# nchopin/particles

Hardware: NVIDIA H100
Metric: particle-steps/sec (N x T), Bootstrap SV (higher is better)
Workload: dtype f64

## Files before the change

include/smcb.h:

```cpp
#ifndef SMCB_H
#define SMCB_H

#include <stdint.h>

#ifdef __cplusplus
extern "C" {
#endif

#define SMCB_OK 0
#define SMCB_EINVAL (-1)
#define SMCB_ECUDA (-2)
#define SMCB_ENOSYS (-3)

typedef struct smcb_ctx smcb_ctx;

const char *smcb_last_error(void);
int smcb_version(void);

int smcb_create(smcb_ctx **out, int device, uint64_t seed);
int smcb_destroy(smcb_ctx *ctx);
int smcb_set_stream(smcb_ctx *ctx, void *cuda_stream);
int smcb_seed(smcb_ctx *ctx, uint64_t seed);
int64_t smcb_launch_count(const smcb_ctx *ctx);


int smcb_normalise(smcb_ctx *ctx, double *lw, int64_t n, double *W_out, double *stats_out);
int smcb_weights_from_stats(smcb_ctx *ctx, const double *lw, int64_t n, const double *stats, double *W_out);

#define SMCB_LSE_SUM 0
#define SMCB_LSE_MEAN 1
#define SMCB_LSE_ESSL 2
int smcb_lse(smcb_ctx *ctx, int mode, const double *v, const double *W, int64_t n,
             double *out);

int smcb_exp_and_normalise(smcb_ctx *ctx, const double *lw, int64_t n, double *W_out);

int smcb_wmean_and_var(smcb_ctx *ctx, const double *W, const double *x, int64_t n, int d,
                       double *out);

#define SMCB_RS_MULTINOMIAL 0
#define SMCB_RS_STRATIFIED 1
#define SMCB_RS_SYSTEMATIC 2
#define SMCB_RS_RESIDUAL 3
#define SMCB_RS_SSP 4

int smcb_cumsum(smcb_ctx *ctx, const double *w, int64_t n, double *cdf_out);

int smcb_searchsorted(smcb_ctx *ctx, const double *cdf, int64_t n, const double *su,
                      int64_t m, int64_t *A_out);

int64_t smcb_resample_scratch_doubles(int64_t n, int64_t m);
int smcb_resample(smcb_ctx *ctx, int scheme, const double *W, int64_t n, int64_t m,
                  int64_t *A_out, const double *u_in, double *scratch);

int smcb_gather(smcb_ctx *ctx, const double *X, int64_t n, const int64_t *A, int64_t m,
                int d, double *Xp);
int smcb_gather_rows(smcb_ctx *ctx, const double *X, int64_t n, const int64_t *A, int64_t m,
                     int d, double *Xp);

int smcb_normal_rvs(smcb_ctx *ctx, const double *loc, double loc0, const double *scale,
                    double scale0, const double *z_in, double *out, int64_t n);
int smcb_normal_logpdf(smcb_ctx *ctx, const double *x, double x0, const double *loc,
                       double loc0, const double *scale, double scale0, double *out,
                       int64_t n);
int smcb_logpdf1(smcb_ctx *ctx, int kind, const double *x, double x0, double p0, double c0, const double *p1,
                 double p10, const double *p2, double p20, double *out, int64_t n);
int smcb_mvnormal_rvs(smcb_ctx *ctx, const double *loc, const double *loc0,
                      const double *scale, const double *scale0, const double *L, int d,
                      const double *z_in, double *out, int64_t n);
int smcb_mvnormal_logpdf(smcb_ctx *ctx, const double *x, const double *loc,
                         const double *loc0, const double *scale, const double *scale0,
                         const double *L, int d, double *out, int64_t n);
int smcb_standard_normal(smcb_ctx *ctx, double *out, int64_t n);
int smcb_uniform(smcb_ctx *ctx, double *out, int64_t n);

int smcb_logistic_target(smcb_ctx *ctx, const double *theta, int64_t n, int d, const double *data,
                         int64_t n_data, double prior_scale, double epn, double *lprior,
                         double *llik, double *lpost);
int smcb_rw_propose(smcb_ctx *ctx, const double *theta, int64_t n, int d, const double *L_dev,
                    const double *z_in, double *prop);
int smcb_mh_accept(smcb_ctx *ctx, int64_t n, int d, double *theta, double *lprior, double *llik,
                   double *lpost, const double *theta_p, const double *lprior_p, const double *llik_p,
                   const double *lpost_p, const double *u_in, double *mean_acc);

int smcb_logistic_wf_move(smcb_ctx *ctx, int64_t M, int d, int P, const double *theta0,
                          const double *lprior0, const double *llik0, const double *lpost0,
                          const double *data, int64_t n_data, double prior_scale, double epn,
                          const double *L_dev, const double *z_in, const double *u_in,
                          double *theta_out, double *lprior_out, double *llik_out, double *lpost_out,
                          double *pb_out);

int smcb_next_annealing_epn(smcb_ctx *ctx, const double *llik, int64_t n, double epn, double alpha, double *out_dev);
int smcb_rw_calibrate(smcb_ctx *ctx, const double *W, const double *theta, int64_t n, int d, double scale,
                      double *L_out);

int smcb_essl_grid(smcb_ctx *ctx, const double *llik, int64_t n, double lo, double hi, const double *max_dev,
                   double *out32_dev);
int smcb_wcov_sums(smcb_ctx *ctx, const double *W, const double *theta, int64_t n, int d, const double *mean_dev,
                   double *out_dev);
int smcb_chol_from_sums(smcb_ctx *ctx, const double *tri_dev, const double *sw_dev, int d, double scale, double *L_out);

int smcb_device_math(smcb_ctx *ctx, int fn, const double *x, double *out, int64_t n);

#define SMCB_FK_BOOTSTRAP 0
#define SMCB_FK_GUIDED 1
#define SMCB_FK_APF 2
#define SMCB_FK_AUXBOOT 3

#define SMCB_MODEL_STOCHVOL 0
#define SMCB_MODEL_LINGAUSS 1
#define SMCB_MODEL_GORDON 2
#define SMCB_MODEL_THETALOGISTIC 3
#define SMCB_MODEL_BEARINGS 4
#define SMCB_MODEL_MVLINGAUSS 5
#define SMCB_MODEL_DISCRETECOX 6
#define SMCB_MODEL_STOCHVOLLEV 7

#define SMCB_MAX_PARAMS 256
#define SMCB_SUMMARY_STRIDE 4

typedef struct smcb_filter smcb_filter;

typedef struct {
    int32_t model, fk, scheme, dim;
    int32_t dy, n_params;
    int32_t world, rank;
    int64_t n;
    int64_t n_global;
    int64_t index_offset;
    int64_t T;
    double essrmin;
    uint64_t seed;
    double params[SMCB_MAX_PARAMS];
    double *X[2];
    double *lw[2];
    int64_t *A;
    double *cdf;
    double *data;
    double *summaries;
    const double *z_in;
    const double *u_in;
    double *scratch;
    const double *step_consts;
    double *local_stats;
    const double *gathered;
    double *mail_local;
    double *mail_peer[8];
    int32_t rs_global, reserved0;
    double *moments;
    double *reserved1;
    const double *peer_X0[8];
    const double *peer_X1[8];
    const double *peer_cdf[8];
} smcb_filter_desc;

int smcb_filter_create(smcb_ctx *ctx, const smcb_filter_desc *desc, smcb_filter **out);
int smcb_filter_destroy(smcb_filter *f);
int smcb_filter_step(smcb_filter *f, int64_t nsteps);
int smcb_filter_step_local(smcb_filter *f);
int smcb_filter_step_finish(smcb_filter *f);
int smcb_p2p_alloc(smcb_ctx *ctx, int64_t bytes, void **dev_ptr, unsigned char *handle64);
int smcb_p2p_open(smcb_ctx *ctx, const unsigned char *handle64, void **dev_ptr);
int smcb_p2p_close(void *peer_ptr);
int smcb_p2p_free(void *dev_ptr);
int smcb_filter_step_timed(smcb_filter *f, int64_t nsteps, double *out8);
int smcb_filter_state(smcb_filter *f, double *out8);

#define SMCB_SMOOTH_ON2 0
#define SMCB_SMOOTH_MCMC 1
#define SMCB_SMOOTH_REJECT 2
#define SMCB_SMOOTH_GATHER 3

typedef struct {
    int32_t method, model, dim, n_params;
    int64_t T, N, M;
    int64_t nsteps;
    int64_t max_trials;
    double params[SMCB_MAX_PARAMS];
    const double *step_consts;
    const double *const *X;
    const double *const *lw;
    const int64_t *const *A;
    int64_t x_stride_n, x_stride_c;
    const double *log_bound;
    const double *cdf;
    int64_t cdf_ld;
    const int64_t *idx_T;
    const double *u;
    const int64_t *prop;
    const double *lu;
    const double *u_exact;
    int64_t *idx;
    double *paths;
    int64_t *counts;
} smcb_smooth_desc;

int smcb_backward_sample(smcb_ctx *ctx, const smcb_smooth_desc *desc);

#ifdef __cplusplus
}
#endif
#endif
```

particles_b200/_lib.py:

```python
import ctypes as C
import os

HERE = os.path.dirname(os.path.abspath(__file__))
SO_PATH = os.environ.get("SMCB_LIB") or os.path.join(HERE, "libsmcb.so")

SMCB_MAX_PARAMS = 256
SUMMARY_STRIDE = 4

RS_CODES = {"multinomial": 0, "stratified": 1, "systematic": 2, "residual": 3, "ssp": 4}
FUSED_SCHEMES = ("multinomial", "stratified", "systematic")
FK_BOOTSTRAP, FK_GUIDED, FK_APF, FK_AUXBOOT = 0, 1, 2, 3
MODEL_STOCHVOL, MODEL_LINGAUSS, MODEL_GORDON, MODEL_THETALOGISTIC = 0, 1, 2, 3
MODEL_BEARINGS, MODEL_MVLINGAUSS, MODEL_DISCRETECOX, MODEL_STOCHVOLLEV = 4, 5, 6, 7
LSE_SUM, LSE_MEAN, LSE_ESSL = 0, 1, 2

c_dp = C.c_void_p


class FilterDesc(C.Structure):
    _fields_ = [
        ("model", C.c_int32), ("fk", C.c_int32), ("scheme", C.c_int32), ("dim", C.c_int32),
        ("dy", C.c_int32), ("n_params", C.c_int32), ("world", C.c_int32), ("rank", C.c_int32),
        ("n", C.c_int64), ("n_global", C.c_int64), ("index_offset", C.c_int64), ("T", C.c_int64),
        ("essrmin", C.c_double), ("seed", C.c_uint64),
        ("params", C.c_double * SMCB_MAX_PARAMS),
        ("X", c_dp * 2), ("lw", c_dp * 2), ("A", c_dp), ("cdf", c_dp), ("data", c_dp),
        ("summaries", c_dp), ("z_in", c_dp), ("u_in", c_dp), ("scratch", c_dp),
        ("step_consts", c_dp), ("local_stats", c_dp), ("gathered", c_dp),
        ("mail_local", c_dp), ("mail_peer", c_dp * 8),
        ("rs_global", C.c_int32), ("reserved0", C.c_int32), ("moments", c_dp), ("reserved1", c_dp),
        ("peer_X0", c_dp * 8), ("peer_X1", c_dp * 8), ("peer_cdf", c_dp * 8),
    ]


SMOOTH_ON2, SMOOTH_MCMC, SMOOTH_REJECT, SMOOTH_GATHER = 0, 1, 2, 3


class SmoothDesc(C.Structure):
    _fields_ = [
        ("method", C.c_int32), ("model", C.c_int32), ("dim", C.c_int32), ("n_params", C.c_int32),
        ("T", C.c_int64), ("N", C.c_int64), ("M", C.c_int64), ("nsteps", C.c_int64), ("max_trials", C.c_int64),
        ("params", C.c_double * SMCB_MAX_PARAMS), ("step_consts", c_dp),
        ("X", c_dp), ("lw", c_dp), ("A", c_dp), ("x_stride_n", C.c_int64), ("x_stride_c", C.c_int64),
        ("log_bound", c_dp), ("cdf", c_dp), ("cdf_ld", C.c_int64), ("idx_T", c_dp),
        ("u", c_dp), ("prop", c_dp), ("lu", c_dp), ("u_exact", c_dp),
        ("idx", c_dp), ("paths", c_dp), ("counts", c_dp),
    ]


PROTOTYPES = {
    "smcb_last_error": (C.c_char_p, []),
    "smcb_version": (C.c_int, []),
    "smcb_create": (C.c_int, [C.POINTER(C.c_void_p), C.c_int, C.c_uint64]),
    "smcb_destroy": (C.c_int, [C.c_void_p]),
    "smcb_set_stream": (C.c_int, [C.c_void_p, C.c_void_p]),
    "smcb_seed": (C.c_int, [C.c_void_p, C.c_uint64]),
    "smcb_launch_count": (C.c_int64, [C.c_void_p]),
    "smcb_normalise": (C.c_int, [C.c_void_p, c_dp, C.c_int64, c_dp, c_dp]),
    "smcb_weights_from_stats": (C.c_int, [C.c_void_p, c_dp, C.c_int64, c_dp, c_dp]),
    "smcb_lse": (C.c_int, [C.c_void_p, C.c_int, c_dp, c_dp, C.c_int64, c_dp]),
    "smcb_exp_and_normalise": (C.c_int, [C.c_void_p, c_dp, C.c_int64, c_dp]),
    "smcb_wmean_and_var": (C.c_int, [C.c_void_p, c_dp, c_dp, C.c_int64, C.c_int, c_dp]),
    "smcb_cumsum": (C.c_int, [C.c_void_p, c_dp, C.c_int64, c_dp]),
    "smcb_searchsorted": (C.c_int, [C.c_void_p, c_dp, C.c_int64, c_dp, C.c_int64, c_dp]),
    "smcb_resample_scratch_doubles": (C.c_int64, [C.c_int64, C.c_int64]),
    "smcb_resample": (C.c_int, [C.c_void_p, C.c_int, c_dp, C.c_int64, C.c_int64, c_dp, c_dp, c_dp]),
    "smcb_gather": (C.c_int, [C.c_void_p, c_dp, C.c_int64, c_dp, C.c_int64, C.c_int, c_dp]),
    "smcb_gather_rows": (C.c_int, [C.c_void_p, c_dp, C.c_int64, c_dp, C.c_int64, C.c_int, c_dp]),
    "smcb_normal_rvs": (C.c_int, [C.c_void_p, c_dp, C.c_double, c_dp, C.c_double, c_dp, c_dp, C.c_int64]),
    "smcb_normal_logpdf": (C.c_int, [C.c_void_p, c_dp, C.c_double, c_dp, C.c_double, c_dp, C.c_double,
                                     c_dp, C.c_int64]),
    "smcb_logpdf1": (C.c_int, [C.c_void_p, C.c_int, c_dp, C.c_double, C.c_double, C.c_double, c_dp, C.c_double, c_dp,
                               C.c_double, c_dp, C.c_int64]),
    "smcb_mvnormal_rvs": (C.c_int, [C.c_void_p, c_dp, c_dp, c_dp, c_dp, c_dp, C.c_int, c_dp, c_dp, C.c_int64]),
    "smcb_mvnormal_logpdf": (C.c_int, [C.c_void_p, c_dp, c_dp, c_dp, c_dp, c_dp, c_dp, C.c_int, c_dp,
                                       C.c_int64]),
    "smcb_standard_normal": (C.c_int, [C.c_void_p, c_dp, C.c_int64]),
    "smcb_uniform": (C.c_int, [C.c_void_p, c_dp, C.c_int64]),
    "smcb_logistic_target": (C.c_int, [C.c_void_p, c_dp, C.c_int64, C.c_int, c_dp, C.c_int64, C.c_double,
                                       C.c_double, c_dp, c_dp, c_dp]),
    "smcb_logistic_wf_move": (C.c_int, [C.c_void_p, C.c_int64, C.c_int, C.c_int, c_dp, c_dp, c_dp, c_dp, c_dp,
                                        C.c_int64, C.c_double, C.c_double, c_dp, c_dp, c_dp, c_dp, c_dp, c_dp,
                                        c_dp, c_dp]),
    "smcb_rw_propose": (C.c_int, [C.c_void_p, c_dp, C.c_int64, C.c_int, c_dp, c_dp, c_dp]),
    "smcb_mh_accept": (C.c_int, [C.c_void_p, C.c_int64, C.c_int, c_dp, c_dp, c_dp, c_dp, c_dp, c_dp, c_dp, c_dp,
                                 c_dp, c_dp]),
    "smcb_next_annealing_epn": (C.c_int, [C.c_void_p, c_dp, C.c_int64, C.c_double, C.c_double, c_dp]),
    "smcb_rw_calibrate": (C.c_int, [C.c_void_p, c_dp, c_dp, C.c_int64, C.c_int, C.c_double, c_dp]),
    "smcb_essl_grid": (C.c_int, [C.c_void_p, c_dp, C.c_int64, C.c_double, C.c_double, c_dp, c_dp]),
    "smcb_wcov_sums": (C.c_int, [C.c_void_p, c_dp, c_dp, C.c_int64, C.c_int, c_dp, c_dp]),
    "smcb_chol_from_sums": (C.c_int, [C.c_void_p, c_dp, c_dp, C.c_int, C.c_double, c_dp]),
    "smcb_device_math": (C.c_int, [C.c_void_p, C.c_int, c_dp, c_dp, C.c_int64]),
    "smcb_filter_create": (C.c_int, [C.c_void_p, C.POINTER(FilterDesc), C.POINTER(C.c_void_p)]),
    "smcb_filter_destroy": (C.c_int, [C.c_void_p]),
    "smcb_filter_step": (C.c_int, [C.c_void_p, C.c_int64]),
    "smcb_filter_step_local": (C.c_int, [C.c_void_p]),
    "smcb_filter_step_finish": (C.c_int, [C.c_void_p]),
    "smcb_p2p_alloc": (C.c_int, [C.c_void_p, C.c_int64, C.POINTER(C.c_void_p), C.c_char_p]),
    "smcb_p2p_open": (C.c_int, [C.c_void_p, C.c_char_p, C.POINTER(C.c_void_p)]),
    "smcb_p2p_close": (C.c_int, [C.c_void_p]),
    "smcb_p2p_free": (C.c_int, [C.c_void_p]),
    "smcb_filter_step_timed": (C.c_int, [C.c_void_p, C.c_int64, C.POINTER(C.c_double)]),
    "smcb_filter_state": (C.c_int, [C.c_void_p, C.POINTER(C.c_double)]),
    "smcb_backward_sample": (C.c_int, [C.c_void_p, C.POINTER(SmoothDesc)]),
}

_lib = None


class SmcbError(RuntimeError):
    pass


def load():
    global _lib
    if _lib is None:
        if not os.path.exists(SO_PATH):
            raise SmcbError(
                f"{SO_PATH} is missing: build it with `python -m particles_b200.build` "
                "(there is no CPU fallback for this path)")
        lib = C.CDLL(SO_PATH)
        for name, (res, args) in PROTOTYPES.items():
            fn = getattr(lib, name)
            fn.restype, fn.argtypes = res, args
        _lib = lib
    return _lib


def check(rc):
    if rc == 0:
        return
    msg = load().smcb_last_error().decode()
    if rc == -1:
        raise ValueError(msg)
    if rc == -3:
        raise NotImplementedError(msg)
    raise SmcbError(msg)
```

particles_b200/core.py:

```python
import ctypes as C
import time

import numpy as np
import torch

from . import _lib
from . import collectors
from . import resampling as rs
from .device import as_device, context, empty, ptr, require_cuda, tensor_from_ptr


class FeynmanKac:

    def __init__(self, T):
        self.T = T

    def _error_msg(self, meth):
        return f"method/property {meth} missing in class {self.__class__.__name__}"

    def M0(self, N):
        raise NotImplementedError(self._error_msg("M0"))

    def M(self, t, xp):
        raise NotImplementedError(self._error_msg("M"))

    def logG(self, t, xp, x):
        raise NotImplementedError(self._error_msg("logG"))

    @property
    def isAPF(self):
        return "logeta" in dir(self)

    def done(self, smc):
        return smc.t >= self.T

    def time_to_resample(self, smc):
        return smc.aux.ESS < smc.N * smc.ESSrmin

    def default_moments(self, W, X):
        return rs.wmean_and_var(W, X)

    def summary_format(self, smc):
        return "t=%i: resample:%s, ESS (end of iter)=%.2f" % (smc.t, smc.rs_flag, smc.wgts.ESS)


def _is_apf(fk):
    return fk.isAPF if hasattr(fk, "isAPF") else ("logeta" in dir(fk))


class _FusedEngine:

    def __init__(self, spec, N, scheme, ESSrmin, seed, noise=None, n_global=None, index_offset=0,
                 world=1, rank=0, group=None, p2p=False, global_rs=False, moments=False):
        self.world, self.rank, self.group = int(world), int(rank), group
        self.p2p = bool(p2p) and self.world > 1
        self.global_rs = bool(global_rs) and self.world > 1
        if self.global_rs and not self.p2p:
            raise ValueError("global resampling over shards needs the peer-memory exchange (exchange='p2p')")
        self._pool = None
        self.ctx = context()
        self.lib = self.ctx.lib
        self.N, self.T = int(N), int(spec["data"].shape[0])
        n, T = self.N, self.T
        self.dim, self.dy = int(spec.get("dim", 1)), int(spec.get("dy", 1))
        dev = self.ctx.device
        f64 = dict(dtype=torch.float64, device=dev)
        xshape = (n,) if self.dim == 1 else (self.dim, n)
        if self.p2p:
            self._pool = _p2p_pool(self.ctx, self.world, self.rank, group)
        if self.global_rs:
            arena = self._pool.arena((2 * self.dim + 1) * n * 8)
            nd = self.dim * n
            self.X = [tensor_from_ptr(arena, xshape, owner=self._pool), tensor_from_ptr(arena + nd * 8, xshape, owner=self._pool)]
            self.cdf = tensor_from_ptr(arena + 2 * nd * 8, (n,), owner=self._pool)
        else:
            self.X = [torch.empty(xshape, **f64), torch.empty(xshape, **f64)]
            self.cdf = torch.empty(n, **f64)
        self.lw = [torch.empty(n, **f64), torch.empty(n, **f64)]
        self.A = torch.empty(n, dtype=torch.int64, device=dev)
        self.summ = torch.zeros((T, _lib.SUMMARY_STRIDE), **f64)
        self.mom = torch.zeros((T, 8), **f64) if moments else None
        self.data_host = torch.from_numpy(spec["data"].reshape(-1)).pin_memory()
        self.data = self.data_host.to(dev, non_blocking=True)
        self.sc = None
        if spec.get("step_consts") is not None:
            self.sc = as_device(spec["step_consts"])
        self.scratch = torch.empty(n + 2, **f64) if scheme == "multinomial" else None
        self.z_in = self.u_in = None
        if noise is not None:
            z, u = noise
            self.z_in = None if z is None else as_device(z)
            self.u_in = None if u is None else as_device(u)
        d = _lib.FilterDesc()
        d.model, d.fk, d.scheme, d.dim = spec["model"], spec["fk"], _lib.RS_CODES[scheme], self.dim
        d.dy, d.n_params = self.dy, len(spec["params"])
        d.n, d.n_global = n, int(n_global or n)
        d.index_offset, d.T = int(index_offset), T
        d.essrmin, d.seed = float(ESSrmin), int(seed) & (2 ** 64 - 1)
        for i, v in enumerate(spec["params"]):
            d.params[i] = float(v)
        d.X[0], d.X[1] = self.X[0].data_ptr(), self.X[1].data_ptr()
        d.lw[0], d.lw[1] = self.lw[0].data_ptr(), self.lw[1].data_ptr()
        d.A, d.cdf = self.A.data_ptr(), self.cdf.data_ptr()
        d.data, d.summaries = self.data.data_ptr(), self.summ.data_ptr()
        d.z_in = self.z_in.data_ptr() if self.z_in is not None else None
        d.u_in = self.u_in.data_ptr() if self.u_in is not None else None
        d.scratch = self.scratch.data_ptr() if self.scratch is not None else None
        d.step_consts = self.sc.data_ptr() if self.sc is not None else None
        d.moments = self.mom.data_ptr() if self.mom is not None else None
        d.world, d.rank = self.world, self.rank
        if self.world > 1:
            self.local_stats = torch.zeros(16, **f64)
            self.gathered = torch.zeros(16 * self.world, **f64)
            d.local_stats, d.gathered = self.local_stats.data_ptr(), self.gathered.data_ptr()
            if self.p2p:
                mail = self._pool.mailbox()
                d.mail_local = mail[self.rank]
                for r in range(self.world):
                    d.mail_peer[r] = mail[r]
            if self.global_rs:
                nd = self.dim * n * 8
                d.rs_global = 1
                for r in range(self.world):
                    base = self._pool.arena_of(r)
                    d.peer_X0[r], d.peer_X1[r], d.peer_cdf[r] = base, base + nd, base + 2 * nd
        self.desc = d
        h = C.c_void_p()
        _lib.check(self.lib.smcb_filter_create(self.ctx.handle, C.byref(d), C.byref(h)))
        self.handle = h

    def step(self, nsteps=1):
        self.ctx.bind_stream()
        if self.world == 1 or self.p2p:
            _lib.check(self.lib.smcb_filter_step(self.handle, int(nsteps)))
            return
        import torch.distributed as dist
        for _ in range(int(nsteps)):
            _lib.check(self.lib.smcb_filter_step_local(self.handle))
            dist.all_gather_into_tensor(self.gathered, self.local_stats, group=self.group)
            _lib.check(self.lib.smcb_filter_step_finish(self.handle))

    def step_timed(self, nsteps):
        self.ctx.bind_stream()
        out = (C.c_double * 8)()
        _lib.check(self.lib.smcb_filter_step_timed(self.handle, int(nsteps), out))
        ms = dict(zip(("init", "step_rs", "tail", "step"), out[0:4]))
        cnt = dict(zip(("init", "step_rs", "tail", "step"), (int(v) for v in out[4:8])))
        return ms, cnt

    def state(self):
        out = (C.c_double * 8)()
        _lib.check(self.lib.smcb_filter_state(self.handle, out))
        return list(out)

    def close(self):
        if getattr(self, "handle", None):
            self.lib.smcb_filter_destroy(self.handle)
            self.handle = None

    def __del__(self):
        try:
            self.close()
        except Exception:
            pass


class _P2PPool:

    def __init__(self, ctx, world, rank, group):
        self.ctx, self.lib, self.world, self.rank, self.group = ctx, ctx.lib, world, rank, group
        self._mail = None
        self._arena = None
        self._arena_bytes = 0
        self._gen = 0

    def _exchange(self, nbytes):
        import torch.distributed as dist
        ptr_ = C.c_void_p()
        hbuf = C.create_string_buffer(64)
        _lib.check(self.lib.smcb_p2p_alloc(self.ctx.handle, int(nbytes), C.byref(ptr_), hbuf))
        mine = torch.frombuffer(bytearray(hbuf.raw), dtype=torch.uint8).to(self.ctx.device)
        allh = torch.empty(64 * self.world, dtype=torch.uint8, device=self.ctx.device)
        dist.all_gather_into_tensor(allh, mine, group=self.group)
        allh = allh.cpu().numpy().tobytes()
        out = []
        for r in range(self.world):
            if r == self.rank:
                out.append(ptr_.value)
                continue
            pp = C.c_void_p()
            _lib.check(self.lib.smcb_p2p_open(self.ctx.handle, allh[64 * r:64 * (r + 1)], C.byref(pp)))
            out.append(pp.value)
        return out

    def mailbox(self):
        nslab, slab = 4, 2 * self.world * 32 * 8
        if self._mail is None:
            self._mail = self._exchange(nslab * slab)
        g = self._gen
        self._gen += 1
        tensor_from_ptr(self._mail[self.rank] + ((g + 2) % nslab) * slab, (slab // 8,), owner=self).zero_()
        return [p + (g % nslab) * slab for p in self._mail]

    def arena(self, nbytes):
        if self._arena is None or nbytes > self._arena_bytes:
            self._arena = self._exchange(nbytes)
            self._arena_bytes = nbytes
        return self._arena[self.rank]

    def arena_of(self, r):
        return self._arena[r]


_pools = {}


def _p2p_pool(ctx, world, rank, group):
    key = (ctx.device.index, id(group) if group is not None else None, world, rank)
    if key not in _pools:
        _pools[key] = _P2PPool(ctx, world, rank, group)
    return _pools[key]


class SMC:

    def __init__(self, fk=None, N=100, qmc=False, resampling="systematic", ESSrmin=0.5,
                 store_history=False, verbose=False, collect=None, seed=None, fused=None,
                 noise=None):
        require_cuda()
        _lib.load()
        if qmc:
            raise NotImplementedError("SQMC (qmc=True) is outside the accelerated path")
        if resampling not in rs.rs_funcs:
            raise ValueError(f"{resampling} is not a valid resampling scheme")
        self.fk, self.N, self.qmc = fk, N, qmc
        self.resampling, self.ESSrmin, self.verbose = resampling, ESSrmin, verbose
        self.t = 0
        self._done = 0
        self.cpu_time = None
        self.summaries = None if collect == "off" else collectors.Summaries(collect)
        self._seed = np.random.randint(0, 2 ** 31 - 1) if seed is None else int(seed)
        self._engine = None
        self._dev_moments = False
        self._noise = noise
        spec = None
        if fused is not False:
            from .state_space_models import fused_spec
            spec = fused_spec(fk)
            if spec is not None and resampling not in _lib.FUSED_SCHEMES:
                spec = None
            if spec is None and fused is True:
                raise NotImplementedError("this Feynman-Kac model has no fused kernel")
        if spec is not None:
            self._dev_moments = self.summaries is not None and self.summaries.device_moments(fk)
            self._engine = _FusedEngine(spec, N, resampling, ESSrmin, self._seed, noise,
                                        moments=self._dev_moments)
            self._row_cache = {}
        else:
            context().seed(self._seed)
            self._p = {"rs_flag": False, "logLt": 0.0, "wgts": rs.Weights(), "aux": None,
                       "X": None, "Xp": None, "A": None}
        from . import smoothing
        self.hist = smoothing.generate_hist_obj(store_history, self)

    @property
    def fused(self):
        return self._engine is not None

    def _row(self, t):
        if t not in self._row_cache:
            self._row_cache = {t: self._engine.summ[t].cpu().numpy()}
        return self._row_cache[t]

    def _cur(self):
        return (self._done - 1) & 1

    @property
    def X(self):
        if not self.fused:
            return self._p["X"]
        if self._done == 0:
            return None
        x = self._engine.X[self._cur()]
        return x if x.ndim == 1 else x.t()

    @X.setter
    def X(self, v):
        self._p["X"] = v

    @property
    def rs_flag(self):
        if not self.fused:
            return self._p["rs_flag"]
        return False if self._done == 0 else bool(self._row(self._done - 1)[2])

    @property
    def logLt(self):
        if not self.fused:
            return self._p["logLt"]
        return 0.0 if self._done == 0 else float(self._row(self._done - 1)[1])

    @property
    def log_mean_w(self):
        if not self.fused:
            return self._p["log_mean_w"]
        return float(self._row(self._done - 1)[3])

    @property
    def loglt(self):
        if not self.fused:
            return self._p["loglt"]
        t = self._done - 1
        if t == 0 or self.rs_flag:
            return self.log_mean_w
        return self.log_mean_w - float(self._engine.summ[t - 1, 3].item())

    @property
    def A(self):
        if not self.fused:
            return self._p["A"]
        if self._done <= 1:
            return None
        if self.rs_flag:
            return self._engine.A
        return torch.arange(self.N, device=self._engine.A.device)

    @property
    def Xp(self):
        if not self.fused:
            return self._p["Xp"]
        if self._done <= 1:
            return None
        prev = self._engine.X[self._cur() ^ 1]
        if not self.rs_flag:
            return prev if prev.ndim == 1 else prev.t()
        out = torch.empty_like(prev)
        ctx = self._engine.ctx
        _lib.check(ctx.lib.smcb_gather(ctx.handle, ptr(prev), self.N, ptr(self._engine.A), self.N,
                                       self._engine.dim, ptr(out)))
        return out if out.ndim == 1 else out.t()

    @property
    def wgts(self):
        if not self.fused:
            return self._p["wgts"]
        if self._done == 0:
            return rs.Weights()
        st = self._engine.state()
        stats = torch.tensor([st[6], st[5], st[4], st[7]], dtype=torch.float64,
                             device=self._engine.lw[0].device)
        return rs.Weights._from_device_stats(self._engine.lw[self._cur()], stats)

    @property
    def aux(self):
        if not self.fused:
            return self._p["aux"]
        return self.wgts

    @property
    def W(self):
        return self.wgts.W

    def __str__(self):
        return self.fk.summary_format(self)

    def reset_weights(self):
        p = self._p
        if _is_apf(self.fk):
            lw = rs.log_mean_exp(self.logetat, W=p["wgts"].W) - self._gather(self.logetat, p["A"])
            p["wgts"] = rs.Weights(lw=lw)
        else:
            p["wgts"] = rs.Weights()

    def setup_auxiliary_weights(self):
        p = self._p
        if _is_apf(self.fk):
            self.logetat = as_device(self.fk.logeta(self.t - 1, p["X"]))
            p["aux"] = p["wgts"].add(self.logetat)
        else:
            p["aux"] = p["wgts"]

    def _gather(self, X, A):
        if not isinstance(X, (torch.Tensor, np.ndarray)):
            return X[A]
        ctx = context()
        X = as_device(X)
        d = 1 if X.ndim == 1 else X.shape[1]
        out = torch.empty((A.shape[0],) + tuple(X.shape[1:]), dtype=X.dtype, device=X.device)
        _lib.check(ctx.lib.smcb_gather_rows(ctx.handle, ptr(X), X.shape[0], ptr(A), A.shape[0], d,
                                            ptr(out)))
        return out

    def generate_particles(self):
        self._p["X"] = self.fk.M0(self.N)

    def reweight_particles(self):
        p = self._p
        p["wgts"] = p["wgts"].add(self.fk.logG(self.t, p["Xp"], p["X"]))

    def resample_move(self):
        p = self._p
        p["rs_flag"] = bool(self.fk.time_to_resample(self))
        if p["rs_flag"]:
            p["A"] = rs.resampling(self.resampling, p["aux"].W, M=self.N)
            p["Xp"] = self._gather(p["X"], p["A"])
            self.reset_weights()
        else:
            p["A"] = torch.arange(self.N, device="cuda")
            p["Xp"] = p["X"]
        p["X"] = self.fk.M(self.t, p["Xp"])

    def compute_summaries(self):
        p = self._p
        if self.t > 0:
            prec = p["log_mean_w"]
        p["log_mean_w"] = p["wgts"].log_mean
        if self.t == 0 or p["rs_flag"]:
            p["loglt"] = p["log_mean_w"]
        else:
            p["loglt"] = p["log_mean_w"] - prec
        p["logLt"] += p["loglt"]
        if self.verbose:
            print(self)
        if self.hist:
            self.hist.save(self)
        if self.summaries:
            self.summaries.collect(self)

    def __next__(self):
        if self.fk.done(self):
            raise StopIteration
        if self.fused:
            self._engine.step(1)
            self._done += 1
            if self.verbose:
                print(self)
            if self.hist:
                self.hist.save(self)
            if self.summaries:
                self.summaries.collect(self)
            self.t += 1
            return
        if self.t == 0:
            self.generate_particles()
        else:
            self.setup_auxiliary_weights()
            self.resample_move()
        self.reweight_particles()
        self.compute_summaries()
        self.t += 1
        self._done = self.t

    def next(self):
        return self.__next__()

    def __iter__(self):
        return self

    def run(self):
        t0 = time.perf_counter()
        if self.fused and not self.verbose and not self.hist \
                and (self.summaries is None or self.summaries.only_defaults or self._dev_moments) \
                and getattr(getattr(type(self.fk), "done", None), "__qualname__", "") == "FeynmanKac.done":
            T = self._engine.T
            first = self.t
            if first < T:
                self._engine.step(T - first)
                self.t = self._done = T
            table = self._engine.summ.cpu().numpy()
            self._row_cache = {T - 1: table[T - 1]}
            if self.summaries is not None:
                self.summaries._extend_defaults([float(v) for v in table[first:T, 0]],
                                                [float(v) for v in table[first:T, 1]],
                                                [bool(v) for v in table[first:T, 2]])
                if self._dev_moments:
                    self.summaries._extend_moments(self._engine.mom.cpu().numpy()[first:T], self._engine.dim)
        else:
            for _ in self:
                pass
            if self.fused:
                torch.cuda.synchronize()
        self.cpu_time = time.perf_counter() - t0
```

particles_b200/csrc/smcb_filter.cu:

```cuda
#include <stdlib.h>

#include "smcb_step.cuh"

int smcb_bind_nd(smcb_filter *f);
int smcb_bind_1d_more(smcb_filter *f);

static int smcb_bind_1d(smcb_filter *f) {
    const smcb_filter_desc *d = &f->desc;
    switch (d->model) {
        case SMCB_MODEL_STOCHVOL: return bind_fk<StochVolM>(f);
        case SMCB_MODEL_LINGAUSS: return bind_fk<LinGaussM>(f);
        case SMCB_MODEL_GORDON:
        case SMCB_MODEL_THETALOGISTIC:
        case SMCB_MODEL_DISCRETECOX:
        case SMCB_MODEL_STOCHVOLLEV: return smcb_bind_1d_more(f);
        default:
            set_error("fused filter: model id %d is not available in the fused 1-D family", d->model);
            return SMCB_ENOSYS;
    }
}

static int filter_setup(smcb_filter *f, smcb_ctx *c, const smcb_filter_desc *d);

extern "C" int smcb_filter_create(smcb_ctx *c, const smcb_filter_desc *d, smcb_filter **out) {
    SMCB_REQUIRE(c && d && out, "smcb_filter_create: NULL argument");
    SMCB_REQUIRE(d->n >= 1 && d->T >= 1, "smcb_filter_create: need n >= 1 and T >= 1");
    SMCB_REQUIRE(d->X[0] && d->X[1] && d->lw[0] && d->lw[1] && d->A && d->cdf && d->data && d->summaries,
                 "smcb_filter_create: NULL device buffer");
    SMCB_REQUIRE((d->index_offset & 1) == 0, "smcb_filter_create: index_offset must be even");
    SMCB_REQUIRE(d->dim >= 1 && d->dim <= 4, "smcb_filter_create: fused kernels exist for state dimension 1..4 (dim=%d)", d->dim);
    SMCB_REQUIRE(d->dy >= 1 && d->dy <= kMaxDy, "smcb_filter_create: observation dimension must be 1..%d", kMaxDy);
    SMCB_REQUIRE(d->essrmin >= 0.0 && d->essrmin <= 1.0, "smcb_filter_create: ESSrmin must be in [0, 1]");
    smcb_filter *f = new (std::nothrow) smcb_filter();
    SMCB_REQUIRE(f != nullptr, "smcb_filter_create: out of host memory");
    f->ctx = c;
    f->desc = *d;
    f->t_host = 0;
    f->timed = false;
    f->mem = nullptr;
    const int rc = filter_setup(f, c, d);
    if (rc) {
        if (f->mem) cudaFree(f->mem);
        delete f;
        return rc;
    }
    *out = f;
    return SMCB_OK;
}

static bool env_flag(const char *name, bool dflt) {
    const char *v = getenv(name);
    if (!v || !*v) return dflt;
    return v[0] != '0';
}

static int filter_setup(smcb_filter *f, smcb_ctx *c, const smcb_filter_desc *d) {
    int rc = (d->dim == 1) ? smcb_bind_1d(f) : smcb_bind_nd(f);
    if (rc) return rc;

    const int64_t n = d->n;
    constexpr size_t kHdr = 512;
    static_assert(2 * sizeof(StepState) <= 384, "StepState outgrew its header slot");
    const size_t part = (size_t)2 * kMaxStepGrid * kPartStride * sizeof(double);
    const size_t agg = (size_t)(kMaxStepGrid + 8) * sizeof(double);
    SMCB_CUDA(cudaMalloc(&f->mem, kHdr + part + agg));
    SMCB_CUDA(cudaMemsetAsync(f->mem, 0, kHdr + part + agg, c->stream));
    FilterArgs &a = f->args;
    memset(&a, 0, sizeof(a));
    a.st = reinterpret_cast<StepState *>(f->mem);
    a.bar = reinterpret_cast<unsigned long long *>(f->mem + 384);
    a.sync_timeout = reinterpret_cast<int *>(f->mem + 392);
    a.partials = reinterpret_cast<double *>(f->mem + kHdr);
    a.blk_agg = reinterpret_cast<double *>(f->mem + kHdr + part);
    a.math_tab = c->math_tab;
    a.X[0] = d->X[0]; a.X[1] = d->X[1]; a.lw[0] = d->lw[0]; a.lw[1] = d->lw[1];
    a.A = reinterpret_cast<long long *>(d->A);
    a.cdf = d->cdf;
    a.su = (d->scheme == SMCB_RS_MULTINOMIAL) ? d->scratch : nullptr;
    SMCB_REQUIRE(d->scheme != SMCB_RS_MULTINOMIAL || d->scratch != nullptr,
                 "smcb_filter_create: multinomial needs desc.scratch of n + 2 doubles");
    a.data = d->data;
    a.sc = d->step_consts;
    a.summaries = d->summaries;
    a.moments = d->moments;
    a.z_in = d->z_in; a.u_in = d->u_in;
    a.dy = d->dy;
    a.n = n; a.n_global = d->n_global > 0 ? d->n_global : n;
    a.index_offset = d->index_offset; a.T = d->T;
    a.essrmin = d->essrmin;
    a.key = key_of(d->seed);
    {
        int dev = 0, sms = kSMs;
        SMCB_CUDA(cudaGetDevice(&dev));
        SMCB_CUDA(cudaDeviceGetAttribute(&sms, cudaDevAttrMultiProcessorCount, dev));
        const int64_t npairs = (n + 1) / 2;
        int64_t g = sms < kMaxStepGrid ? sms : kMaxStepGrid;
        const int64_t gmax = (npairs + f->block_size - 1) / f->block_size;
        if (g > gmax) g = gmax;
        if (g < 1) g = 1;
        int64_t chunk = (npairs + g - 1) / g;
        g = (npairs + chunk - 1) / chunk;
        a.chunk = chunk;
        f->grid_move = (int)g;
        a.grid = f->grid_move;
        const bool apf = d->fk == SMCB_FK_APF || d->fk == SMCB_FK_AUXBOOT;
        const bool mom = d->moments != nullptr;
        a.slab_lane = (!apf && !mom) ? 1 : 0;
        a.slab_stride = a.slab_lane ? 96 : 4 + (apf ? 4 : 0) + (mom ? 2 * d->dim : 0);
        const int64_t cap = f->slab_doubles / a.slab_stride;
        const int64_t n_iter = (chunk + f->pairs_per_iteration - 1) / f->pairs_per_iteration;
        int64_t slab_it = 2, n_small = 0;
        for (;; slab_it++) {
            const int64_t ns = (cap * slab_it - n_iter) / (slab_it - 1) - 1;
            const int64_t want = n_iter < 32 ? n_iter : 32;
            if (ns >= want) { n_small = ns < 0 ? 0 : (ns > n_iter / 8 ? n_iter / 8 : ns); break; }
        }
        if (n_small > n_iter) n_small = n_iter;
        a.slab_it = (int)slab_it;
        a.slab_small = (int)n_small;
    }
    a.world = d->world > 1 ? d->world : 1;
    a.rank = d->world > 1 ? d->rank : 0;
    a.local_stats = d->local_stats;
    a.gathered = d->gathered;
    a.mail_local = (a.world > 1) ? d->mail_local : nullptr;
    for (int r = 0; r < 8; r++) a.mail_peer[r] = (a.world > 1 && r < a.world) ? d->mail_peer[r] : nullptr;
    SMCB_REQUIRE(a.world == 1 || (a.rank >= 0 && a.rank < a.world), "smcb_filter_create: bad rank");
    SMCB_REQUIRE(a.world == 1 || a.mail_local || (d->local_stats && d->gathered),
                 "smcb_filter_create: world > 1 needs either a peer mailbox or local_stats / gathered");
    SMCB_REQUIRE(a.world <= 8, "smcb_filter_create: at most 8 ranks");
    if (a.mail_local) {
        for (int r = 0; r < a.world; r++)
            SMCB_REQUIRE(a.mail_peer[r] != nullptr, "smcb_filter_create: mail_peer[%d] is NULL", r);
    }
    a.rs_global = (a.world > 1 && d->rs_global) ? 1 : 0;
    if (a.rs_global) {
        SMCB_REQUIRE(a.mail_local != nullptr, "smcb_filter_create: global resampling needs the peer mailbox");
        SMCB_REQUIRE((n & 1) == 0, "smcb_filter_create: global resampling needs an even shard size");
        if (d->scheme != SMCB_RS_SYSTEMATIC && d->scheme != SMCB_RS_STRATIFIED) {
            set_error("fused filter: global resampling over shards supports systematic and stratified");
            return SMCB_ENOSYS;
        }
        for (int r = 0; r < a.world; r++) {
            SMCB_REQUIRE(d->peer_X0[r] && d->peer_X1[r] && d->peer_cdf[r],
                         "smcb_filter_create: peer_X0 / peer_X1 / peer_cdf[%d] is NULL", r);
            a.pX[r][0] = d->peer_X0[r]; a.pX[r][1] = d->peer_X1[r]; a.pcdf[r] = d->peer_cdf[r];
        }
    }
    f->pdl = env_flag("SMCB_PDL", true);
    f->coop = env_flag("SMCB_COOP", false);
    return SMCB_OK;
}

extern "C" int smcb_filter_destroy(smcb_filter *f) {
    if (!f) return SMCB_OK;
    cudaStreamSynchronize(f->ctx->stream);
    cudaFree(f->mem);
    delete f;
    return SMCB_OK;
}

static int launch_one(smcb_filter *f) {
    if (f->t_host >= f->desc.T) {
        set_error("smcb_filter_step: all %lld steps already done (StopIteration)", (long long)f->desc.T);
        return SMCB_EINVAL;
    }
    int rc = (f->t_host == 0) ? f->launch_init(f) : f->launch_step(f);
    if (rc && f->t_host > 0 && (f->pdl || f->coop)) {
        cudaGetLastError();
        f->pdl = false; f->coop = false;
        rc = f->launch_step(f);
    }
    if (rc) return rc;
    f->t_host++;
    return SMCB_OK;
}

extern "C" int smcb_filter_step_local(smcb_filter *f) {
    SMCB_REQUIRE(f != nullptr && f->args.world > 1 && f->args.mail_local == nullptr,
                 "smcb_filter_step_local: not a sharded filter with the host-driven exchange");
    int rc = launch_one(f);
    if (rc) return rc;
    return f->launch_publish(f);
}

extern "C" int smcb_filter_step_finish(smcb_filter *f) {
    SMCB_REQUIRE(f != nullptr && f->args.world > 1, "smcb_filter_step_finish: not a sharded filter");
    return f->launch_tail(f);
}

extern "C" int smcb_filter_step(smcb_filter *f, int64_t nsteps) {
    SMCB_REQUIRE(f != nullptr, "smcb_filter_step: NULL filter");
    SMCB_REQUIRE(f->args.world == 1 || f->args.mail_local != nullptr,
                 "smcb_filter_step: sharded filters without a peer mailbox use step_local / step_finish");
    if (nsteps <= 0) return SMCB_OK;
    for (int64_t i = 0; i < nsteps; i++) {
        int rc = launch_one(f);
        if (rc) return rc;
    }
    return f->launch_tail(f);
}

extern "C" int smcb_filter_step_timed(smcb_filter *f, int64_t nsteps, double *out8) {
    SMCB_REQUIRE(f && out8, "smcb_filter_step_timed: NULL argument");
    SMCB_REQUIRE(nsteps >= 1 && nsteps <= 100000, "smcb_filter_step_timed: nsteps out of range");
    SMCB_REQUIRE(f->t_host + nsteps <= f->desc.T, "smcb_filter_step_timed: past the last step");
    SMCB_REQUIRE(f->args.world == 1, "smcb_filter_step_timed: single-device filters only");
    cudaStream_t s = f->ctx->stream;
    const size_t nev = (size_t)(nsteps + 1) * 2;
    cudaEvent_t *ev = new (std::nothrow) cudaEvent_t[nev];
    double *rows = new (std::nothrow) double[(size_t)nsteps * SMCB_SUMMARY_STRIDE];
    size_t made = 0;
    int rc = SMCB_OK;
    const int64_t t_first = f->t_host;
    auto fail = [&](cudaError_t e, const char *what) {
        set_error("smcb_filter_step_timed: %s -> %s", what, cudaGetErrorString(e));
        rc = SMCB_ECUDA;
    };
    if (!ev || !rows) { set_error("smcb_filter_step_timed: out of host memory"); rc = SMCB_EINVAL; }
    for (; rc == SMCB_OK && made < nev; made++) {
        cudaError_t e = cudaEventCreate(&ev[made]);
        if (e != cudaSuccess) { fail(e, "cudaEventCreate"); break; }
    }
    f->timed = true;
    for (int64_t i = 0; rc == SMCB_OK && i <= nsteps; i++) {
        cudaEventRecord(ev[2 * i], s);
        rc = (i < nsteps) ? launch_one(f) : f->launch_tail(f);
        cudaEventRecord(ev[2 * i + 1], s);
    }
    f->timed = false;
    if (rc == SMCB_OK) {
        cudaError_t e = cudaStreamSynchronize(s);
        if (e != cudaSuccess) fail(e, "cudaStreamSynchronize");
    }
    if (rc == SMCB_OK) {
        cudaError_t e = cudaMemcpy(rows, f->args.summaries + (size_t)t_first * SMCB_SUMMARY_STRIDE,
                                   sizeof(double) * nsteps * SMCB_SUMMARY_STRIDE, cudaMemcpyDeviceToHost);
        if (e != cudaSuccess) fail(e, "cudaMemcpy(summaries)");
    }
    if (rc == SMCB_OK) {
        for (int j = 0; j < 8; j++) out8[j] = 0.0;
        for (int64_t i = 0; i <= nsteps; i++) {
            float ms = 0.f;
            cudaEventElapsedTime(&ms, ev[2 * i], ev[2 * i + 1]);
            int kind = 2;
            if (i < nsteps) {
                const int64_t t = t_first + i;
                kind = (t == 0) ? 0 : (rows[(size_t)i * SMCB_SUMMARY_STRIDE + 2] != 0.0 ? 1 : 3);
            }
            out8[kind] += ms;
            out8[4 + kind] += 1.0;
        }
    }
    for (size_t i = 0; i < made; i++) cudaEventDestroy(ev[i]);
    delete[] ev;
    delete[] rows;
    return rc;
}

extern "C" int smcb_filter_state(smcb_filter *f, double *out8) {
    SMCB_REQUIRE(f && out8, "smcb_filter_state: NULL argument");
    SMCB_REQUIRE(f->t_host >= 1, "smcb_filter_state: no step has run yet");
    struct { StepState st[2]; char pad[384 - 2 * sizeof(StepState)]; unsigned long long bar; int timeout; int pad2; } h;
    static_assert(sizeof(h) == 400, "header snapshot layout");
    SMCB_CUDA(cudaMemcpyAsync(&h, f->mem, sizeof(h), cudaMemcpyDeviceToHost, f->ctx->stream));
    SMCB_CUDA(cudaStreamSynchronize(f->ctx->stream));
    const StepState &s = h.st[(f->t_host - 1) & 1];
    out8[0] = (double)(s.t + 1); out8[1] = (double)((f->t_host - 1) & 1); out8[2] = (double)s.rs; out8[3] = s.logLt;
    out8[4] = s.ess; out8[5] = s.log_mean_w; out8[6] = s.wm; out8[7] = s.ws;
    if (h.timeout) {
        set_error(h.timeout == 2 ? "fused filter: the grid barrier of a resampling step timed out (the step kernel was "
                                   "not co-resident: another kernel occupies the device)"
                                 : "sharded filter: a wait on a peer GPU's flag timed out (a rank died or fell out of step)");
        return SMCB_ECUDA;
    }
    if (s.t != f->t_host - 1) {
        set_error("smcb_filter_state: the last step is not finalised (internal error: t=%lld, expected %lld)",
                  (long long)s.t, (long long)(f->t_host - 1));
        return SMCB_ECUDA;
    }
    return SMCB_OK;
}

extern "C" int smcb_p2p_alloc(smcb_ctx *c, int64_t bytes, void **dev_ptr, unsigned char *handle64) {
    SMCB_REQUIRE(c && dev_ptr && handle64 && bytes > 0, "smcb_p2p_alloc: bad argument");
    static_assert(sizeof(cudaIpcMemHandle_t) == 64, "IPC handle size");
    void *p = nullptr;
    SMCB_CUDA(cudaMalloc(&p, (size_t)bytes));
    SMCB_CUDA(cudaMemset(p, 0, (size_t)bytes));
    cudaIpcMemHandle_t h;
    SMCB_CUDA(cudaIpcGetMemHandle(&h, p));
    memcpy(handle64, &h, 64);
    *dev_ptr = p;
    return SMCB_OK;
}

extern "C" int smcb_p2p_open(smcb_ctx *c, const unsigned char *handle64, void **dev_ptr) {
    SMCB_REQUIRE(c && dev_ptr && handle64, "smcb_p2p_open: bad argument");
    cudaIpcMemHandle_t h;
    memcpy(&h, handle64, 64);
    SMCB_CUDA(cudaIpcOpenMemHandle(dev_ptr, h, cudaIpcMemLazyEnablePeerAccess));
    return SMCB_OK;
}

extern "C" int smcb_p2p_close(void *peer_ptr) {
    if (peer_ptr) SMCB_CUDA(cudaIpcCloseMemHandle(peer_ptr));
    return SMCB_OK;
}

extern "C" int smcb_p2p_free(void *dev_ptr) {
    if (dev_ptr) SMCB_CUDA(cudaFree(dev_ptr));
    return SMCB_OK;
}
```

particles_b200/csrc/smcb_step.cuh:

```cuda
#pragma once
#include <string.h>

#include <new>

#include "smcb_common.cuh"
#include "smcb_math.cuh"
#include "smcb_models.cuh"
#include "smcb_scan.cuh"
#include "smcb_search.cuh"

using namespace smcb;

namespace smcb {

constexpr int kPartStride = 16;
constexpr int kMailStride = 32;
constexpr int kMailEpoch = 16;
constexpr int kMailScan = 17;
constexpr int kMaxStepGrid = 256;
constexpr int kMaxD = 4;
constexpr int kTailBlock = 256;
#ifndef SMCB_SPECULATE
#define SMCB_SPECULATE 1
#endif
template <class M> struct StepCfg {
    static constexpr int BS = 512;
    static constexpr int kU = (M::D == 1) ? 2 : 1;
    static constexpr int kStage = 8 * BS;
    static constexpr int kSlabRecords = 128;
    static constexpr int kSlabDoubles = kSlabRecords * 96;
    static constexpr size_t dyn_smem = kMathTabBytes + (size_t)(2 * kStage > kSlabDoubles ? 2 * kStage : kSlabDoubles) * sizeof(double);
};
constexpr int kScanGroupWarps = 2;
constexpr int kMovePairs = 2;

struct StepState {
    double logLt, log_mean_w, ess;
    double wm, ws, wq;
    long long t;
    long long nrs;
    int rs;
    int rs_next;
    int pad[2];
};

struct FilterArgs {
    double *X[2];
    double *lw[2];
    long long *A;
    double *cdf;
    double *su;
    const double *data;
    const double *sc;
    double *summaries;
    double *moments;
    const double *z_in, *u_in;
    StepState *st;
    int *sync_timeout;
    double *partials;
    unsigned long long *bar;
    double *blk_agg;
    const double *math_tab;
    int slab_it;
    int slab_small;
    int slab_lane;
    int slab_stride;
    int64_t n, n_global, index_offset, T;
    int dy;
    int world, rank;
    int grid;
    int64_t chunk;
    double essrmin;
    Philox key;
    double *local_stats;
    const double *gathered;
    double *mail_local;
    double *mail_peer[8];
    int rs_global;
    const double *pX[8][2];
    const double *pcdf[8];
};

__device__ __forceinline__ void wait_epoch(const volatile double *flag, double epoch, int *timeout) {
    const long long t0 = clock64();
    if (*reinterpret_cast<volatile int *>(timeout)) return;
    while (*flag < epoch) {
        if (clock64() - t0 > 8000000000ll) { *timeout = 1; break; }
    }
    __threadfence_system();
}

__device__ __forceinline__ StepK step_consts(const FilterArgs &a, long long t) {
    StepK k;
    k.t = t;
#pragma unroll
    for (int i = 0; i < kMaxDy; i++) {
        k.yv[i] = (i < a.dy && t >= 0) ? a.data[t * a.dy + i] : 0.0;
        k.yn[i] = (i < a.dy && t + 1 < a.T) ? a.data[(t + 1) * a.dy + i] : 0.0;
    }
    k.y = k.yv[0];
    k.y_next = k.yn[0];
    k.sc0 = (a.sc && t >= 0) ? a.sc[t] : 0.0;
    return k;
}

__device__ __forceinline__ double fix_nan(double v) { return v != v ? -CUDART_INF : v; }

__device__ __forceinline__ void weights_scalars(const Lse3 &a, double n, double &log_mean, double &ess) {
    if (a.m == -CUDART_INF || a.m == CUDART_INF || a.m != a.m) {
        log_mean = CUDART_NAN;
        ess = CUDART_NAN;
        return;
    }
    log_mean = a.m + log(a.s / n);
    ess = (a.s * a.s) / a.q;
}

__device__ __forceinline__ double shift_factor(double m, double M) {
    return (m == -CUDART_INF) ? 0.0 : fexp_neg(m - M);
}

__device__ __forceinline__ double nanmax(double a, double b) { return (b > a || b != b) ? b : a; }

template <int NV, int BS, bool MAX>
__device__ __forceinline__ void block_reduce_all(double (&v)[NV], double *smem) {
    constexpr int NWARP = BS / 32;
    static_assert(NWARP <= 32, "one lane per warp in the second level");
    const int lane = threadIdx.x & 31, warp = threadIdx.x >> 5;
#pragma unroll
    for (int j = 0; j < NV; j++) {
#pragma unroll
        for (int mask = 16; mask > 0; mask >>= 1) {
            const double o = __shfl_xor_sync(0xffffffffu, v[j], mask);
            v[j] = MAX ? nanmax(v[j], o) : v[j] + o;
        }
    }
    if (lane == 0) {
#pragma unroll
        for (int j = 0; j < NV; j++) smem[warp * NV + j] = v[j];
    }
    __syncthreads();
    if (warp == 0) {
#pragma unroll
        for (int j = 0; j < NV; j++) {
            double x = (lane < NWARP) ? smem[lane * NV + j] : (MAX ? -CUDART_INF : 0.0);
#pragma unroll
            for (int mask = 16; mask > 0; mask >>= 1) {
                const double o = __shfl_xor_sync(0xffffffffu, x, mask);
                x = MAX ? nanmax(x, o) : x + o;
            }
            if (lane == 0) smem[NWARP * NV + j] = x;
        }
    }
    __syncthreads();
#pragma unroll
    for (int j = 0; j < NV; j++) v[j] = smem[NWARP * NV + j];
    __syncthreads();
}
template <int NV, int BS>
__device__ __forceinline__ void block_max_all(double (&v)[NV], double *smem) { block_reduce_all<NV, BS, true>(v, smem); }
template <int NV, int BS>
__device__ __forceinline__ void block_sum_all(double (&v)[NV], double *smem) { block_reduce_all<NV, BS, false>(v, smem); }

template <int D>
struct Acc {
    Lse3 w;
    double sx[D], sxx[D];
};

template <int D>
__device__ __forceinline__ void acc_init(Acc<D> &a) {
    a.w = lse3_empty();
#pragma unroll
    for (int c = 0; c < D; c++) { a.sx[c] = 0.0; a.sxx[c] = 0.0; }
}

template <int NV, int D, bool FINITE, bool MOM>
__device__ __forceinline__ void acc_add_batch_t(Acc<D> &a, const double (&v)[NV], const double (&x)[NV][D]) {
    double mb = v[0];
#pragma unroll
    for (int j = 1; j < NV; j++) mb = FINITE ? (v[j] > mb ? v[j] : mb) : fmax(mb, v[j]);
    if (mb > a.w.m) {
        const double r = texp_neg(a.w.m - mb);
        a.w.s *= r;
        a.w.q *= r * r;
        if (MOM) {
#pragma unroll
            for (int c = 0; c < D; c++) { a.sx[c] *= r; a.sxx[c] *= r; }
        }
        a.w.m = mb;
    }
    if (!FINITE && a.w.m == -CUDART_INF) return;
#pragma unroll
    for (int j = 0; j < NV; j++) {
        const double e = FINITE ? texp_sat(v[j] - a.w.m) : texp_neg(v[j] - a.w.m);
        a.w.s += e;
        a.w.q = fma(e, e, a.w.q);
        if (MOM && (FINITE || v[j] != -CUDART_INF)) {
#pragma unroll
            for (int c = 0; c < D; c++) {
                const double ex = e * x[j][c];
                a.sx[c] += ex;
                a.sxx[c] = fma(ex, x[j][c], a.sxx[c]);
            }
        }
    }
}
template <int NV, int D, bool FINITE = false>
__device__ __forceinline__ void acc_add_batch(Acc<D> &a, const double (&v)[NV], const double (&x)[NV][D], bool mom) {
    if (mom) acc_add_batch_t<NV, D, FINITE, true>(a, v, x);
    else acc_add_batch_t<NV, D, FINITE, false>(a, v, x);
}

struct StepSmem {
    double red[32 * 16];
    int next;
    double ringP[32];
    int ringF[32];
    double gwarp[16][8];
    double gpref[16][2];
    int gqn[16];
    long long gq[16][8][3];
    int *timeout_ptr;
    double peer[8][kMailStride];
    double goff[9], gpi[8];
    double pref[2];
    double carry[20];
};

__device__ __forceinline__ double shift_factor_t(double m, double M) {
    return (m == -CUDART_INF) ? 0.0 : texp_neg(m - M);
}

__device__ __forceinline__ double warp_max_nan(double v) {
#pragma unroll
    for (int mask = 16; mask > 0; mask >>= 1) {
        const double o = __shfl_xor_sync(0xffffffffu, v, mask);
        v = (o > v || o != o) ? o : v;
    }
    return v;
}
__device__ __forceinline__ double warp_sum(double v) {
#pragma unroll
    for (int mask = 16; mask > 0; mask >>= 1) v += __shfl_xor_sync(0xffffffffu, v, mask);
    return v;
}

template <int D, bool APF>
__device__ __forceinline__ void warp_reduce_to_slab(const Acc<D> &sa, const Lse3 &sx, bool mom, double *rec, int lane) {
    const double M = warp_max_nan(sa.w.m);
    const double e = shift_factor_t(sa.w.m, M);
    const double s = warp_sum(sa.w.s * e), q = warp_sum(sa.w.q * (e * e));
    if (lane == 0) { rec[0] = M; rec[1] = s; rec[2] = q; }
    int off = 4;
    if (APF) {
        const double Ma = warp_max_nan(sx.m);
        const double ea = shift_factor_t(sx.m, Ma);
        const double as_ = warp_sum(sx.s * ea), aq = warp_sum(sx.q * (ea * ea));
        if (lane == 0) { rec[4] = Ma; rec[5] = as_; rec[6] = aq; }
        off = 8;
    }
    if (mom) {
#pragma unroll
        for (int c = 0; c < D; c++) {
            const double a1 = warp_sum(sa.sx[c] * e), a2 = warp_sum(sa.sxx[c] * e);
            if (lane == 0) { rec[off + c] = a1; rec[off + D + c] = a2; }
        }
    }
}

template <int D, bool APF, int BS>
__device__ __forceinline__ void write_partial(const FilterArgs &a, long long t, const Acc<D> &acc, const Lse3 &aux,
                                              bool mom, StepSmem &sh, const double *s_slab = nullptr, int n_slab = 0) {
    const bool lane_rec = a.slab_lane != 0;
    const int n_rec = lane_rec ? n_slab * 32 : n_slab;
    auto rec_ptr = [&](int r) {
        return lane_rec ? s_slab + (size_t)(r >> 5) * a.slab_stride + (r & 31) : s_slab + (size_t)r * a.slab_stride;
    };
    const int rs_ = lane_rec ? 32 : 1;
    if (n_slab > 0) __syncthreads();
    double mx[2] = {acc.w.m, APF ? aux.m : -CUDART_INF};
    for (int r = threadIdx.x; r < n_rec; r += BS) {
        const double *rec = rec_ptr(r);
        mx[0] = nanmax(mx[0], rec[0]);
        if (APF && !lane_rec) mx[1] = nanmax(mx[1], rec[4]);
    }
    block_max_all<2, BS>(mx, sh.red);
    const double ew = shift_factor_t(acc.w.m, mx[0]);
    const double ea = APF ? shift_factor_t(aux.m, mx[1]) : 0.0;
    double v[4 + 2 * D];
    v[0] = acc.w.s * ew;
    v[1] = acc.w.q * (ew * ew);
    v[2] = APF ? aux.s * ea : 0.0;
    v[3] = APF ? aux.q * (ea * ea) : 0.0;
#pragma unroll
    for (int c = 0; c < D; c++) {
        v[4 + c] = mom ? acc.sx[c] * ew : 0.0;
        v[4 + D + c] = mom ? acc.sxx[c] * ew : 0.0;
    }
    for (int r = threadIdx.x; r < n_rec; r += BS) {
        const double *rec = rec_ptr(r);
        const double e = shift_factor_t(rec[0], mx[0]);
        v[0] += rec[rs_] * e;
        v[1] += rec[2 * rs_] * (e * e);
        if (!lane_rec) {
            if (APF) {
                const double e2 = shift_factor_t(rec[4], mx[1]);
                v[2] += rec[5] * e2;
                v[3] += rec[6] * (e2 * e2);
            }
            if (mom) {
                const int off = APF ? 8 : 4;
#pragma unroll
                for (int c = 0; c < D; c++) { v[4 + c] += rec[off + c] * e; v[4 + D + c] += rec[off + D + c] * e; }
            }
        }
    }
    if (mom) block_sum_all<4 + 2 * D, BS>(v, sh.red);
    else {
        double w4[4] = {v[0], v[1], v[2], v[3]};
        block_sum_all<4, BS>(w4, sh.red);
        v[0] = w4[0]; v[1] = w4[1]; v[2] = w4[2]; v[3] = w4[3];
    }
    if (threadIdx.x == 0) {
        double *p = a.partials + ((size_t)(t & 1) * kMaxStepGrid + blockIdx.x) * kPartStride;
        p[0] = mx[0]; p[1] = v[0]; p[2] = v[1]; p[3] = 0.0;
        p[4] = APF ? mx[1] : mx[0]; p[5] = APF ? v[2] : v[0]; p[6] = APF ? v[3] : v[1]; p[7] = 0.0;
#pragma unroll
        for (int c = 0; c < kMaxD; c++) {
            p[8 + c] = (c < D) ? v[4 + (c < D ? c : 0)] : 0.0;
            p[12 + c] = (c < D) ? v[4 + D + (c < D ? c : 0)] : 0.0;
        }
    }
}

__device__ __forceinline__ void merge16(double (&a)[16], const double *b) {
#pragma unroll
    for (int k = 0; k < 2; k++) {
        const double am = a[4 * k], bm = b[4 * k];
        const double M = (bm > am || bm != bm) ? bm : am;
        const double ea = shift_factor(am, M), eb = shift_factor(bm, M);
        a[4 * k] = M;
        a[4 * k + 1] = a[4 * k + 1] * ea + b[4 * k + 1] * eb;
        a[4 * k + 2] = a[4 * k + 2] * (ea * ea) + b[4 * k + 2] * (eb * eb);
        if (k == 0) {
#pragma unroll
            for (int c = 8; c < 16; c++) a[c] = a[c] * ea + b[c] * eb;
        }
    }
}

template <bool APF>
__device__ __forceinline__ void shard_totals(const FilterArgs &a, long long s, bool mom, StepSmem &sh, double (&loc)[16]) {
    const int G = a.grid, tid = threadIdx.x;
    if (tid < 32) {
        const double *base = a.partials + (size_t)(s & 1) * kMaxStepGrid * kPartStride;
        constexpr int kR = kMaxStepGrid / 32;
        double pm[kR], ps[kR], pq[kR], xm[kR], xs[kR], xq[kR];
        double mw = -CUDART_INF, ma = -CUDART_INF;
#pragma unroll
        for (int i = 0; i < kR; i++) {
            const int r = tid + 32 * i;
            pm[i] = -CUDART_INF; ps[i] = 0.0; pq[i] = 0.0; xm[i] = -CUDART_INF; xs[i] = 0.0; xq[i] = 0.0;
            if (r < G) {
                const double *row = base + (size_t)r * kPartStride;
                const double2 r0 = __ldcg(reinterpret_cast<const double2 *>(row));
                pm[i] = r0.x; ps[i] = r0.y; pq[i] = __ldcg(row + 2);
                if (APF) {
                    const double2 r1 = __ldcg(reinterpret_cast<const double2 *>(row + 4));
                    xm[i] = r1.x; xs[i] = r1.y; xq[i] = __ldcg(row + 6);
                }
            }
            mw = nanmax(mw, pm[i]);
            if (APF) ma = nanmax(ma, xm[i]);
        }
        mw = warp_max_nan(mw);
        if (APF) ma = warp_max_nan(ma);
        double v[12];
#pragma unroll
        for (int j2 = 0; j2 < 12; j2++) v[j2] = 0.0;
#pragma unroll
        for (int i = 0; i < kR; i++) {
            const int r = tid + 32 * i;
            const double ew = shift_factor(pm[i], mw);
            v[0] += ps[i] * ew;
            v[1] += pq[i] * (ew * ew);
            if (APF) {
                const double ea = shift_factor(xm[i], ma);
                v[2] += xs[i] * ea;
                v[3] += xq[i] * (ea * ea);
            }
            if (mom && r < G) {
                const double *row = base + (size_t)r * kPartStride + 8;
#pragma unroll
                for (int c = 0; c < 8; c++) v[4 + c] += __ldcg(row + c) * ew;
            }
        }
#pragma unroll
        for (int j2 = 0; j2 < 12; j2++)
            if (j2 < 4 || mom) v[j2] = warp_sum(v[j2]);
        if (tid == 0) {
            double *o = sh.peer[0];
            o[0] = mw; o[1] = v[0]; o[2] = v[1]; o[3] = 0.0;
            o[4] = APF ? ma : mw; o[5] = APF ? v[2] : v[0]; o[6] = APF ? v[3] : v[1]; o[7] = 0.0;
#pragma unroll
            for (int c = 0; c < 8; c++) o[8 + c] = v[4 + c];
        }
    }
    __syncthreads();
#pragma unroll
    for (int j2 = 0; j2 < 16; j2++) loc[j2] = sh.peer[0][j2];
    __syncthreads();
}

template <int BS>
__device__ __forceinline__ void cta_prefix(double v, StepSmem &sh, double &p_b, double &p_next) {
    const int tid = threadIdx.x, lane = tid & 31, warp = tid >> 5;
    const double iw = warp_scan_monotone(v, lane);
    if (lane == 31) sh.red[warp] = iw;
    __syncthreads();
    double woff = 0.0;
    for (int w_ = 0; w_ < BS / 32; w_++)
        if (w_ < warp) woff = woff + sh.red[w_];
    const double incl = woff + iw;
    if (tid == 0 && blockIdx.x == 0) sh.pref[0] = 0.0;
    if (tid + 1 == (int)blockIdx.x) sh.pref[0] = incl;
    if (tid == (int)blockIdx.x) sh.pref[1] = incl;
    __syncthreads();
    p_b = sh.pref[0];
    p_next = fmax(sh.pref[1], p_b);
    __syncthreads();
}

struct StepDecision {
    int rs;
    long long nrs_prev;
    double reset_c;
    double xm, xs;
    double p_b, p_next;
};

struct PrologueCarry {
    bool mom;
};

template <bool APF>
__device__ __forceinline__ bool prologue_begin(const FilterArgs &a, long long t, StepSmem &sh, bool writer,
                                               PrologueCarry &pc) {
    const long long s = t - 1;
    const int tid = threadIdx.x;
    pc.mom = writer && a.moments != nullptr;
    StepState prev;
    prev.logLt = 0.0; prev.log_mean_w = 0.0; prev.nrs = 0; prev.rs_next = 0;
    if (s >= 1) {
        const StepState *pp = a.st + ((s - 1) & 1);
        prev.logLt = __ldcg(&pp->logLt); prev.log_mean_w = __ldcg(&pp->log_mean_w);
        prev.nrs = __ldcg(&pp->nrs); prev.rs_next = __ldcg(&pp->rs_next);
    }
    double loc[16];
    shard_totals<APF>(a, s, pc.mom, sh, loc);
    if (tid == 0) {
#pragma unroll
        for (int i = 0; i < 16; i++) sh.carry[i] = loc[i];
        sh.carry[16] = prev.logLt; sh.carry[17] = prev.log_mean_w;
        sh.carry[18] = __longlong_as_double(prev.nrs); sh.carry[19] = __longlong_as_double((long long)prev.rs_next);
    }
    if (a.world > 1 && a.mail_local != nullptr) {
        if (writer && tid < a.world) {
            double *slot = a.mail_peer[tid] + ((size_t)(s & 1) * a.world + a.rank) * kMailStride;
#pragma unroll
            for (int i = 0; i < 16; i++) slot[i] = loc[i];
            __threadfence_system();
            *reinterpret_cast<volatile double *>(slot + kMailEpoch) = (double)(s + 1);
        }
    }
    const Lse3 xl{loc[4], loc[5], loc[6]};
    double lm_l, ess_l;
    weights_scalars(xl, (double)a.n, lm_l, ess_l);
    return (s + 1 < a.T) && (ess_l < (double)a.n * a.essrmin);
}

template <bool APF, int BS>
__device__ __forceinline__ StepDecision prologue_end(const FilterArgs &a, long long t, StepSmem &sh, bool writer,
                                                     bool need_prefix, const PrologueCarry &pc) {
    const long long s = t - 1;
    const int tid = threadIdx.x;
    __syncthreads();
    StepState prev;
    double loc[16];
#pragma unroll
    for (int i = 0; i < 16; i++) loc[i] = sh.carry[i];
    prev.logLt = sh.carry[16]; prev.log_mean_w = sh.carry[17];
    prev.nrs = __double_as_longlong(sh.carry[18]); prev.rs_next = (int)__double_as_longlong(sh.carry[19]);
    double glob[16];
#pragma unroll
    for (int j = 0; j < 16; j++) glob[j] = loc[j];
    if (a.world > 1) {
        if (a.mail_local != nullptr) {
            const double *box = a.mail_local + (size_t)(s & 1) * a.world * kMailStride;
            if (tid < a.world) {
                wait_epoch(box + (size_t)tid * kMailStride + kMailEpoch, (double)(s + 1), a.sync_timeout);
                for (int i = 0; i < 16; i++)
                    sh.peer[tid][i] = *reinterpret_cast<const volatile double *>(box + (size_t)tid * kMailStride + i);
            }
        } else if (tid < a.world) {
            for (int i = 0; i < 16; i++) sh.peer[tid][i] = __ldcg(a.gathered + (size_t)tid * 16 + i);
        }
        __syncthreads();
#pragma unroll
        for (int j = 0; j < 16; j++) glob[j] = sh.peer[0][j];
        for (int r = 1; r < a.world; r++) merge16(glob, sh.peer[r]);
        if (a.rs_global && tid == 0) {
            double run = 0.0;
            for (int r = 0; r < a.world; r++) {
                const double pm_ = sh.peer[r][4], ps_ = sh.peer[r][5];
                const double pi = (pm_ == -CUDART_INF) ? 0.0 : ps_ * fexp_neg(pm_ - glob[4]) / glob[5];
                sh.goff[r] = run;
                sh.gpi[r] = pi;
                run = run + pi;
            }
            sh.goff[a.world] = run;
        }
        __syncthreads();
    }
    const Lse3 w{glob[0], glob[1], glob[2]}, x{glob[4], glob[5], glob[6]};
    const Lse3 xl{loc[4], loc[5], loc[6]};
    const double N = (double)a.n_global;
    double log_mean, ess, lm_aux, ess_aux;
    weights_scalars(w, N, log_mean, ess);
    if (APF) weights_scalars(x, N, lm_aux, ess_aux);
    else { lm_aux = log_mean; ess_aux = ess; }
    const int rs_s = prev.rs_next;
    const bool fresh = (s == 0) || (rs_s != 0);
    const double loglt = fresh ? log_mean : (log_mean - prev.log_mean_w);
    const double logLt = prev.logLt + loglt;
    StepDecision d;
    d.rs = (s + 1 < a.T) && (ess_aux < N * a.essrmin);
    d.nrs_prev = prev.nrs + (rs_s ? 1 : 0);
    double rc = 0.0;
    if (a.rs_global) rc = APF ? (log(x.s) + x.m) - (log(w.s) + w.m) : 0.0;
    else if (APF || a.world > 1) rc = (log(xl.s) + xl.m) - (log(w.s) + w.m) + log((double)a.world);
    d.reset_c = rc;
    d.xm = xl.m; d.xs = xl.s;
    d.p_b = 0.0; d.p_next = 0.0;
    if (writer && tid == 0) {
        double *row = a.summaries + (size_t)s * SMCB_SUMMARY_STRIDE;
        row[0] = ess; row[1] = logLt; row[2] = (double)rs_s; row[3] = log_mean;
        StepState *o = a.st + (s & 1);
        o->logLt = logLt; o->log_mean_w = log_mean; o->ess = ess;
        o->wm = w.m; o->ws = w.s; o->wq = w.q;
        o->t = s; o->nrs = d.nrs_prev; o->rs = rs_s; o->rs_next = d.rs;
        if (a.moments != nullptr) {
            double *mrow = a.moments + (size_t)s * 2 * kMaxD;
#pragma unroll
            for (int c = 0; c < kMaxD; c++) {
                const double mean = glob[8 + c] / w.s;
                mrow[c] = mean;
                mrow[kMaxD + c] = glob[12 + c] / w.s - mean * mean;
            }
        }
    }
    if (d.rs && need_prefix) {
        double v = 0.0;
        if (tid < a.grid) {
            const double *row = a.partials + ((size_t)(s & 1) * kMaxStepGrid + tid) * kPartStride + (APF ? 4 : 0);
            v = __ldcg(row + 1) * shift_factor(__ldcg(row), d.xm) / d.xs;
        }
        cta_prefix<BS>(v, sh, d.p_b, d.p_next);
    }
    return d;
}

template <bool APF, int BS>
__device__ __forceinline__ StepDecision step_prologue(const FilterArgs &a, long long t, StepSmem &sh, bool writer,
                                                      bool need_prefix) {
    PrologueCarry pc;
    prologue_begin<APF>(a, t, sh, writer, pc);
    return prologue_end<APF, BS>(a, t, sh, writer, need_prefix, pc);
}

__device__ __forceinline__ void grid_barrier(const FilterArgs &a, unsigned long long target) {
    __syncthreads();
    if (threadIdx.x == 0) {
        __threadfence();
        atomicAdd(a.bar, 1ull);
        const long long t0 = clock64();
        while (*reinterpret_cast<volatile unsigned long long *>(a.bar) < target) {
            if (clock64() - t0 > 8000000000ll) { *a.sync_timeout = 2; break; }
        }
        __threadfence();
        asm volatile("fence.proxy.async;" ::: "memory");
    }
    __syncthreads();
}

__device__ __forceinline__ void cta_range(const FilterArgs &a, int64_t &pstart, int64_t &pend) {
    const int64_t npairs = (a.n + 1) >> 1;
    pstart = (int64_t)blockIdx.x * a.chunk;
    pend = pstart + a.chunk < npairs ? pstart + a.chunk : npairs;
    if (pstart > npairs) pstart = npairs;
}

template <class M, int FK>
__global__ void __launch_bounds__(StepCfg<M>::BS, 1) k_init(M model, FilterArgs a) {
    constexpr bool APF = FkTraits<FK>::apf;
    constexpr int D = M::D, NZ = M::NZ, BS = StepCfg<M>::BS;
    __shared__ StepSmem sh;
    __shared__ __align__(8) uint64_t s_tabbar;
    if (threadIdx.x == 0) mtab_issue(a.math_tab, &s_tabbar);
    __syncthreads();
    mbar_wait(&s_tabbar, 0);
    const StepK k = step_consts(a, 0);
    double *Xo = a.X[0], *lwo = a.lw[0];
    Acc<D> acc;
    acc_init(acc);
    Lse3 aux = lse3_empty();
    const bool mom = a.moments != nullptr;
    const int64_t n = a.n;
    const bool has_next = APF && a.T > 1;
    const bool vec_x = (D == 1) || ((n & 1) == 0);
    int64_t pstart, pend;
    cta_range(a, pstart, pend);
    for (int64_t p = pstart + threadIdx.x; p < pend; p += BS) {
        double z[2][NZ], x[2][D], l[2], av[2];
#pragma unroll
        for (int c = 0; c < NZ; c++) {
            if (a.z_in) {
                const double *zz = a.z_in + (size_t)c * n;
                z[0][c] = zz[2 * p];
                z[1][c] = (2 * p + 1 < n) ? zz[2 * p + 1] : 0.0;
            } else {
                normal_pair_tab(a.key, (uint64_t)((a.index_offset >> 1) + p), 0u, (uint32_t)c, z[0][c], z[1][c]);
            }
        }
#pragma unroll
        for (int j = 0; j < 2; j++) {
            double d;
            model_init<M, FK>(model, k, z[j], x[j], d);
            l[j] = fix_nan(d);
            av[j] = has_next ? fix_nan(l[j] + model_logeta<M>(model, k, x[j])) : -CUDART_INF;
        }
        if (2 * p + 1 < n) {
            if (vec_x) {
#pragma unroll
                for (int c = 0; c < D; c++) st2(Xo + (size_t)c * n + 2 * p, x[0][c], x[1][c]);
            } else {
#pragma unroll
                for (int c = 0; c < D; c++) { Xo[(size_t)c * n + 2 * p] = x[0][c]; Xo[(size_t)c * n + 2 * p + 1] = x[1][c]; }
            }
            st2(lwo + 2 * p, l[0], l[1]);
        } else {
#pragma unroll
            for (int c = 0; c < D; c++) { Xo[(size_t)c * n + 2 * p] = x[0][c]; x[1][c] = 0.0; }
            lwo[2 * p] = l[0];
            l[1] = -CUDART_INF; av[1] = -CUDART_INF;
        }
        acc_add_batch<2, D>(acc, l, x, mom);
        if (APF) lse3_add_batch<2>(aux, av);
    }
    write_partial<D, APF, BS>(a, 0, acc, aux, mom, sh);
}

template <class M, int FK>
struct LoadWeights {
    const double *lw, *X;
    int64_t ntot;
    double m, s;
    M model;
    StepK kprev;
    struct Raw { double l[8]; double x[8][FkTraits<FK>::apf ? M::D : 1]; };
    __device__ __forceinline__ void fetch(int64_t i0, int64_t n, Raw &r) const {
        constexpr bool APF = FkTraits<FK>::apf;
        constexpr int D = M::D;
        const bool vec_x = (D == 1) || ((ntot & 1) == 0);
        if (i0 + 8 <= n) {
#pragma unroll
            for (int j = 0; j < 8; j += 2) { double2 t = ld2(lw + i0 + j); r.l[j] = t.x; r.l[j + 1] = t.y; }
            if (APF) {
#pragma unroll
                for (int c = 0; c < D; c++) {
#pragma unroll
                    for (int j = 0; j < 8; j += 2) {
                        if (vec_x) {
                            double2 t = ld2(X + (size_t)c * ntot + i0 + j);
                            r.x[j][APF ? c : 0] = t.x; r.x[j + 1][APF ? c : 0] = t.y;
                        } else {
                            r.x[j][APF ? c : 0] = X[(size_t)c * ntot + i0 + j];
                            r.x[j + 1][APF ? c : 0] = X[(size_t)c * ntot + i0 + j + 1];
                        }
                    }
                }
            }
        } else {
#pragma unroll
            for (int j = 0; j < 8; j++) {
                r.l[j] = (i0 + j < n) ? lw[i0 + j] : -CUDART_INF;
                if (APF) {
#pragma unroll
                    for (int c = 0; c < D; c++) r.x[j][APF ? c : 0] = (i0 + j < n) ? X[(size_t)c * ntot + i0 + j] : 0.0;
                }
            }
        }
    }
    __device__ __forceinline__ void weights(const Raw &r, int64_t i0, int64_t n, double (&v)[8]) const {
        constexpr bool APF = FkTraits<FK>::apf;
        const double inv_s = 1.0 / s;
#pragma unroll
        for (int j = 0; j < 8; j++) {
            double e = r.l[j];
            if (APF) e = fix_nan(e + model_logeta<M>(model, kprev, r.x[j]));
            v[j] = (i0 + j < n) ? texp(e - m) * inv_s : 0.0;
        }
    }
    __device__ __forceinline__ void operator()(int64_t i0, int64_t n, double (&v)[8]) const {
        Raw r;
        fetch(i0, n, r);
        weights(r, i0, n, v);
    }
};

template <int BS, class LOAD>
__device__ __forceinline__ void scan_range(const LOAD &load, int64_t e0, int64_t e1, double p_b, double p_next,
                                           double *out, double *s_warp) {
    const int tid = threadIdx.x, lane = tid & 31, warp = tid >> 5;
    constexpr int kTile = BS * kScanItems;
    double carry = 0.0;
    for (int64_t base0 = e0; base0 < e1; base0 += kTile) {
        const int64_t i0 = base0 + (int64_t)tid * kScanItems;
        double r[kScanItems];
        load(i0, e1, r);
#pragma unroll
        for (int j = 1; j < kScanItems; j++) r[j] = r[j - 1] + r[j];
        const double iw = warp_scan_monotone(r[kScanItems - 1], lane);
        if (lane == 31) s_warp[warp] = iw;
        __syncthreads();
        double woff = 0.0, total = 0.0;
#pragma unroll
        for (int w = 0; w < BS / 32; w++) {
            if (w < warp) woff = woff + s_warp[w];
            total = total + s_warp[w];
        }
        const double incl = woff + iw;
        const double up = __shfl_up_sync(0xffffffffu, iw, 1);
        const double excl = (lane == 0) ? woff : (woff + up);
        const double b_i = fmin(p_b + carry, p_next);
        const double carry_next = carry + total;
        const double b_next = fmin(p_b + carry_next, p_next);
        const double tb = b_i + excl;
        const double cap = fmin(b_i + incl, b_next);
        double o[kScanItems];
#pragma unroll
        for (int j = 0; j < kScanItems; j++) o[j] = fmin(tb + r[j], cap);
        if (i0 + kScanItems <= e1) {
            store_items(out, i0, o);
        } else {
#pragma unroll
            for (int j = 0; j < kScanItems; j++)
                if (i0 + j < e1) out[i0 + j] = o[j];
        }
        carry = carry_next;
        __syncthreads();
    }
}

struct Scatter {
    long long *A;
    double Nd, u;
    long long n_out;
    __device__ __forceinline__ long long F(double c) const {
        const double t = fma(c, Nd, 0.5 - u) + kRintMagic;
        const long long k = (long long)(((unsigned long long)(__double2hiint(t) & 0xFFFFF) << 32) |
                                        (unsigned int)__double2loint(t)) - (1ll << 51);
        return k < 0 ? 0 : (k > n_out ? n_out : k);
    }
};

constexpr int kHeavy = 48;

constexpr int kScanRing = 32;
constexpr int kGroupQ = 8;
__device__ __forceinline__ int *sc_timeout(StepSmem &sh) { return sh.timeout_ptr; }

__device__ __forceinline__ void group_sync(int id, int nthreads) {
    asm volatile("bar.sync %0, %1;" ::"r"(id), "r"(nthreads) : "memory");
}

template <int BS, int GW, class LOAD>
__device__ __forceinline__ void scan_scatter_groups(const LOAD &load, int64_t e0, int64_t e1, double p_b, double p_next,
                                                    double *out, const Scatter &sc, bool last_cta, StepSmem &sh,
                                                    int *s_hint_all, int hint_cap_total) {
    constexpr int NG = BS / 32 / GW, GT = GW * 32, kTile = GT * kScanItems;
    static_assert(NG <= 15 && NG <= kScanRing && GW <= 8, "scan_scatter_groups: one named barrier (ids 1..15) and one table row per group");
    const int tid = threadIdx.x, lane = tid & 31, warp = tid >> 5;
    const int grp = warp / GW, gw = warp % GW, gt = tid - grp * GT;
    int *s_hint = s_hint_all + grp * (hint_cap_total / NG);
    const int hint_cap = hint_cap_total / NG;
    volatile double *ringP = sh.ringP;
    volatile int *ringF = sh.ringF;
    if (tid < kScanRing) { sh.ringF[tid] = (tid == 0) ? 1 : 0; if (tid == 0) sh.ringP[0] = p_b; }
    if (tid < NG) sh.gqn[tid] = 0;
    __syncthreads();
    const int64_t nt = (e1 - e0 + kTile - 1) / kTile;
    typename LOAD::Raw nxt;
    if (grp < nt) load.fetch(e0 + (int64_t)grp * kTile + (int64_t)gt * kScanItems, e1, nxt);
    for (int64_t t = grp; t < nt; t += NG) {
        const int64_t base0 = e0 + t * kTile;
        const int64_t i0 = base0 + (int64_t)gt * kScanItems;
        const bool last_tile = (t == nt - 1);
        double r[kScanItems];
        const typename LOAD::Raw cur = nxt;
        if (t + NG < nt) load.fetch(i0 + (int64_t)NG * kTile, e1, nxt);
        load.weights(cur, i0, e1, r);
#pragma unroll
        for (int j = 1; j < kScanItems; j++) r[j] = r[j - 1] + r[j];
        const double iw = warp_scan_monotone(r[kScanItems - 1], lane);
        if (lane == 31) sh.gwarp[grp][gw] = iw;
        group_sync(grp + 1, GT);
        double woff = 0.0, total = 0.0;
#pragma unroll
        for (int w = 0; w < GW; w++) {
            if (w < gw) woff = woff + sh.gwarp[grp][w];
            total = total + sh.gwarp[grp][w];
        }
        if (gt == 0) {
            const int slot = (int)(t % kScanRing), nslot = (int)((t + 1) % kScanRing);
            const long long t0 = clock64();
            while (ringF[slot] != (int)(t + 1)) {
                if (clock64() - t0 > 4000000000ll) { *sc_timeout(sh) = 3; break; }
            }
            const double Pt = ringP[slot];
            const double Pn = fmin(Pt + total, p_next);
            ringP[nslot] = Pn;
            __threadfence_block();
            ringF[nslot] = (int)(t + 2);
            sh.gpref[grp][0] = Pt;
            sh.gpref[grp][1] = Pn;
        }
        group_sync(grp + 1, GT);
        const double b_i = sh.gpref[grp][0], b_next = sh.gpref[grp][1];
        const double incl = woff + iw;
        const double up = __shfl_up_sync(0xffffffffu, iw, 1);
        const double excl = (lane == 0) ? woff : (woff + up);
        const double tb = b_i + excl;
        const double cap = fmin(b_i + incl, b_next);
        double o[kScanItems];
#pragma unroll
        for (int j = 0; j < kScanItems; j++) o[j] = fmin(tb + r[j], cap);
        if (i0 + kScanItems <= e1) {
            store_items(out, i0, o);
        } else {
#pragma unroll
            for (int j = 0; j < kScanItems; j++)
                if (i0 + j < e1) out[i0 + j] = o[j];
        }
        const long long K0 = (blockIdx.x == 0 && t == 0) ? 0 : sc.F(b_i);
        const long long K1 = (last_tile && last_cta) ? sc.n_out : sc.F(last_tile ? p_next : b_next);
        const bool staged = (K1 - K0) <= (long long)hint_cap;
        if (i0 < e1) {
            const bool tail_thread = (i0 + kScanItems >= e1);
            long long ks = (gt == 0) ? K0 : sc.F(tb);
            const long long kend = (gt == GT - 1 || tail_thread) ? K1 : sc.F(b_i + incl);
            ks = ks < K0 ? K0 : (ks > K1 ? K1 : ks);
#pragma unroll
            for (int j = 0; j < kScanItems; j++) {
                if (i0 + j < e1) {
                    const bool last_entry = (j == kScanItems - 1) || (i0 + j + 1 >= e1);
                    long long ke = last_entry ? kend : sc.F(o[j]);
                    ke = ke < ks ? ks : (ke > kend ? kend : ke);
                    if (staged) {
                        const int rel = gt * kScanItems + j;
                        for (long long k = ks; k < ke; k++) s_hint[(int)(k - K0)] = rel;
                    } else {
                        if (ke - ks > kHeavy) {
                            const int q = atomicAdd(&sh.gqn[grp], 1);
                            if (q < kGroupQ) { sh.gq[grp][q][0] = ks; sh.gq[grp][q][1] = ke; sh.gq[grp][q][2] = i0 + j; ks = ke; }
                        }
                        for (long long k = ks; k < ke; k++) sc.A[k] = i0 + j;
                    }
                    ks = ke;
                }
            }
        }
        group_sync(grp + 1, GT);
        if (staged) {
            const int cnt = (int)(K1 - K0);
            for (int k = gt; k < cnt; k += GT) sc.A[K0 + k] = base0 + s_hint[k];
        } else {
            const int nq = sh.gqn[grp] < kGroupQ ? sh.gqn[grp] : kGroupQ;
            for (int q = 0; q < nq; q++) {
                const long long ks = sh.gq[grp][q][0], ke = sh.gq[grp][q][1], jj = sh.gq[grp][q][2];
                for (long long k = ks + gt; k < ke; k += GT) sc.A[k] = jj;
            }
        }
        group_sync(grp + 1, GT);
        if (gt == 0) sh.gqn[grp] = 0;
    }
    __syncthreads();
}

__device__ __forceinline__ void spacings_range(const FilterArgs &a, int64_t &e0, int64_t &e1) {
    int64_t pstart, pend;
    cta_range(a, pstart, pend);
    e0 = 2 * pstart;
    e1 = 2 * pend < a.n ? 2 * pend : a.n;
    if (blockIdx.x == gridDim.x - 1) e1 = a.n + 1;
}

struct LoadSpacings {
    const double *su;
    __device__ __forceinline__ void operator()(int64_t i0, int64_t n, double (&v)[8]) const {
#pragma unroll
        for (int j = 0; j < 8; j++) v[j] = (i0 + j < n) ? __ldcg(su + i0 + j) : 0.0;
    }
};

template <int BS>
__device__ __forceinline__ void spacings_pass1(const FilterArgs &a, long long t, StepSmem &sh) {
    int64_t e0, e1;
    spacings_range(a, e0, e1);
    const double *uin = a.u_in ? a.u_in + (size_t)t * (a.n + 1) : nullptr;
    double acc[1] = {0.0};
    for (int64_t i = e0 + 2 * (int64_t)threadIdx.x; i < e1; i += 2 * BS) {
        double u0, u1;
        if (uin) { u0 = uin[i]; u1 = (i + 1 < e1) ? uin[i + 1] : 1.0; }
        else uniform_pair(a.key, (uint64_t)(i >> 1), (uint32_t)t, kPurposeUniform, u0, u1);
        const double v0 = -log(u0);
        const double v1 = (i + 1 < e1) ? -log(u1) : 0.0;
        a.su[i] = v0;
        if (i + 1 < e1) a.su[i + 1] = v1;
        acc[0] += v0 + v1;
    }
    block_sum_all<1, BS>(acc, sh.red);
    if (threadIdx.x == 0) a.blk_agg[blockIdx.x] = acc[0];
}

template <int BS>
__device__ __forceinline__ void spacings_pass2(const FilterArgs &a, StepSmem &sh, double *s_warp) {
    const double v = ((int)threadIdx.x < a.grid) ? __ldcg(a.blk_agg + threadIdx.x) : 0.0;
    double p_b, p_next;
    cta_prefix<BS>(v, sh, p_b, p_next);
    int64_t e0, e1;
    spacings_range(a, e0, e1);
    LoadSpacings load{a.su};
    scan_range<BS>(load, e0, e1, p_b, p_next, a.su, s_warp);
}

__device__ __forceinline__ int shard_of(const double *goff, const double *gpi, int world, double su) {
    int k = 0;
    while (k + 1 < world && su >= goff[k + 1]) k++;
    while (k > 0 && !(gpi[k] > 0.0)) k--;
    while (k + 1 < world && !(gpi[k] > 0.0)) k++;
    return k;
}

template <class M, int FK, int SCHEME>
__global__ void __launch_bounds__(StepCfg<M>::BS, 1) k_step(M model, FilterArgs a, long long t) {
    constexpr bool APF = FkTraits<FK>::apf;
    constexpr int D = M::D, NZ = M::NZ, BS = StepCfg<M>::BS;
    constexpr int kStage = StepCfg<M>::kStage;
    extern __shared__ __align__(128) double s_dyn[];
    double *const s_stage = s_dyn + kMathTabDoubles;
    __shared__ StepSmem sh;
    __shared__ double s_su[2];
    __shared__ __align__(8) uint64_t s_bar[2];
    __shared__ __align__(8) uint64_t s_tabbar;
    __shared__ long long s_hi;
    __shared__ double s_warp[BS / 32];
    if (threadIdx.x == 0) { mtab_issue(a.math_tab, &s_tabbar); sh.next = 0; }
    cudaGridDependencySynchronize();
    cudaTriggerProgrammaticLaunchCompletion();
    PrologueCarry pc;
    const bool pred_rs = prologue_begin<APF>(a, t, sh, blockIdx.x == 0, pc);
    const bool speculate = SMCB_SPECULATE && a.world > 1 && a.mail_local != nullptr && !a.rs_global && !pred_rs;
    StepDecision dec;
    dec.rs = 0; dec.nrs_prev = 0; dec.reset_c = 0.0; dec.xm = 0.0; dec.xs = 1.0; dec.p_b = 0.0; dec.p_next = 0.0;
    if (!speculate) dec = prologue_end<APF, BS>(a, t, sh, blockIdx.x == 0, true, pc);
    mbar_wait(&s_tabbar, 0);
    const int cur = (int)((t - 1) & 1);
    const bool rs = dec.rs != 0;
    double reset_c = dec.reset_c;
    const StepK k = step_consts(a, t);
    const StepK kprev = step_consts(a, t - 1);
    const double *__restrict__ Xi = a.X[cur];
    const double *__restrict__ lwi = a.lw[cur];
    double *__restrict__ Xo = a.X[cur ^ 1];
    double *__restrict__ lwo = a.lw[cur ^ 1];
    const int64_t n = a.n;
    const double *zin = a.z_in ? a.z_in + (size_t)t * NZ * n : nullptr;
    const bool last_apf = APF && (t + 1 < a.T);
    const bool mom = a.moments != nullptr;
    const bool vec_x = (D == 1) || ((n & 1) == 0);
    int64_t pstart, pend;
    cta_range(a, pstart, pend);

    Acc<D> acc;
    acc_init(acc);
    Lse3 aux = lse3_empty();
    int n_slab = 0;

    auto do_pair = [&](int64_t p, const double (&xp)[2][D], const double (&base)[2], double (&x)[2][D], double *l,
                       double *av) {
        double z[2][NZ];
#pragma unroll
        for (int c = 0; c < NZ; c++) {
            if (zin) {
                const double *zz = zin + (size_t)c * n;
                z[0][c] = zz[2 * p];
                z[1][c] = (2 * p + 1 < n) ? zz[2 * p + 1] : 0.0;
            } else {
                normal_pair_tab(a.key, (uint64_t)((a.index_offset >> 1) + p), (uint32_t)t, (uint32_t)c,
                                 z[0][c], z[1][c]);
            }
        }
#pragma unroll
        for (int j = 0; j < 2; j++) {
            double d;
            model_move<M, FK>(model, k, xp[j], z[j], x[j], d);
            l[j] = fix_nan(base[j] + d);
            if (APF) av[j] = last_apf ? fix_nan(l[j] + model_logeta<M>(model, k, x[j])) : -CUDART_INF;
        }
        if (2 * p + 1 < n) {
            if (vec_x) {
#pragma unroll
                for (int c = 0; c < D; c++) st2(Xo + (size_t)c * n + 2 * p, x[0][c], x[1][c]);
            } else {
#pragma unroll
                for (int c = 0; c < D; c++) { Xo[(size_t)c * n + 2 * p] = x[0][c]; Xo[(size_t)c * n + 2 * p + 1] = x[1][c]; }
            }
            st2(lwo + 2 * p, l[0], l[1]);
        } else {
#pragma unroll
            for (int c = 0; c < D; c++) { Xo[(size_t)c * n + 2 * p] = x[0][c]; x[1][c] = 0.0; }
            lwo[2 * p] = l[0];
            l[1] = -CUDART_INF;
            if (APF) av[1] = -CUDART_INF;
        }
    };

    if (!rs) {
        constexpr int kU = StepCfg<M>::kU;
        constexpr int kIt = 32 * kU;
        const int lane = threadIdx.x & 31;
        const int npl = (int)(pend - pstart);
        const int n_iter = (npl + kIt - 1) / kIt;
        const int64_t whole = (n >> 1) < pend ? (n >> 1) : pend;
        const int n_full = whole > pstart ? (int)((whole - pstart) / kIt) : 0;
        const bool fast_ok = (zin == nullptr) && vec_x;
        const double *__restrict__ lwi_c = lwi + 2 * pstart;
        const double *__restrict__ Xi_c = Xi + 2 * pstart;
        double *__restrict__ lwo_c = lwo + 2 * pstart;
        double *__restrict__ Xo_c = Xo + 2 * pstart;
        const uint64_t gpair0 = (uint64_t)((a.index_offset >> 1) + pstart);
        struct In { double base[kU][2]; double xp[kU][2][D]; };
        auto load_full = [&](int i, In &in) {
#pragma unroll
            for (int u = 0; u < kU; u++) {
                const int o2 = 2 * (i * kIt + u * 32 + lane);
                const double2 tl = ld2(lwi_c + o2);
                in.base[u][0] = tl.x; in.base[u][1] = tl.y;
#pragma unroll
                for (int c = 0; c < D; c++) {
                    const double2 tx = ld2(Xi_c + (size_t)c * n + o2);
                    in.xp[u][0][c] = tx.x; in.xp[u][1][c] = tx.y;
                }
            }
        };
        auto compute_full = [&](int i, const In &in, Acc<D> &ac, Lse3 &ax) {
            double l[2 * kU], av[APF ? 2 * kU : 1], x[2 * kU][D];
            bool odd = false;
#pragma unroll
            for (int u = 0; u < kU; u++) {
                const int prel = i * kIt + u * 32 + lane;
                double z[2][NZ];
#pragma unroll
                for (int c = 0; c < NZ; c++)
                    normal_pair_tab(a.key, gpair0 + (uint64_t)prel, (uint32_t)t, (uint32_t)c, z[0][c], z[1][c]);
#pragma unroll
                for (int j2 = 0; j2 < 2; j2++) {
                    double d;
                    model_move<M, FK>(model, k, in.xp[u][j2], z[j2], x[2 * u + j2], d);
                    l[2 * u + j2] = in.base[u][j2] + d;
                    odd |= nonfinite(l[2 * u + j2]);
                    if (APF) {
                        av[APF ? 2 * u + j2 : 0] = last_apf ? l[2 * u + j2] + model_logeta<M>(model, k, x[2 * u + j2])
                                                            : -CUDART_INF;
                        odd |= nonfinite(av[APF ? 2 * u + j2 : 0]);
                    }
                }
            }
            if (odd) {
#pragma unroll
                for (int q = 0; q < 2 * kU; q++) {
                    l[q] = fix_nan(l[q]);
                    if (APF) av[APF ? q : 0] = fix_nan(av[APF ? q : 0]);
                }
            }
#pragma unroll
            for (int u = 0; u < kU; u++) {
                const int o2 = 2 * (i * kIt + u * 32 + lane);
#pragma unroll
                for (int c = 0; c < D; c++) st2(Xo_c + (size_t)c * n + o2, x[2 * u][c], x[2 * u + 1][c]);
                st2(lwo_c + o2, l[2 * u], l[2 * u + 1]);
            }
            if (!odd) {
                acc_add_batch<2 * kU, D, true>(ac, l, x, mom);
            } else {
                acc_add_batch<2 * kU, D, false>(ac, l, x, mom);
            }
            if (APF) lse3_add_batch<(APF ? 2 * kU : 1)>(ax, av);
        };
        auto iteration = [&](int i, Acc<D> &ac, Lse3 &ax) {
            double l[2 * kU], av[APF ? 2 * kU : 1], x[2 * kU][D];
            if (fast_ok && i < n_full) {
                In in;
                load_full(i, in);
                compute_full(i, in, ac, ax);
                return;
            }
            double xp[kU][2][D], base[kU][2];
            const int64_t qbase = pstart + (int64_t)i * kIt;
#pragma unroll
            for (int u = 0; u < kU; u++) {
                const int64_t p = qbase + u * 32 + lane;
                if (p < pend && 2 * p + 1 < n) {
                    double2 tl = ld2(lwi + 2 * p);
                    base[u][0] = tl.x; base[u][1] = tl.y;
#pragma unroll
                    for (int c = 0; c < D; c++) {
                        if (vec_x) {
                            double2 tx = ld2(Xi + (size_t)c * n + 2 * p);
                            xp[u][0][c] = tx.x; xp[u][1][c] = tx.y;
                        } else {
                            xp[u][0][c] = Xi[(size_t)c * n + 2 * p]; xp[u][1][c] = Xi[(size_t)c * n + 2 * p + 1];
                        }
                    }
                } else if (p < pend) {
                    base[u][0] = lwi[2 * p]; base[u][1] = 0.0;
#pragma unroll
                    for (int c = 0; c < D; c++) { xp[u][0][c] = Xi[(size_t)c * n + 2 * p]; xp[u][1][c] = 0.0; }
                }
            }
#pragma unroll
            for (int u = 0; u < kU; u++) {
                const int64_t p = qbase + u * 32 + lane;
                if (p < pend) {
                    do_pair(p, xp[u], base[u], reinterpret_cast<double (&)[2][D]>(x[2 * u]), l + 2 * u,
                            APF ? av + 2 * u : av);
                } else {
                    l[2 * u] = l[2 * u + 1] = -CUDART_INF;
                    if (APF) av[APF ? 2 * u : 0] = av[APF ? 2 * u + 1 : 0] = -CUDART_INF;
#pragma unroll
                    for (int c = 0; c < D; c++) { x[2 * u][c] = 0.0; x[2 * u + 1][c] = 0.0; }
                }
            }
            acc_add_batch<2 * kU, D>(ac, l, x, mom);
            if (APF) lse3_add_batch<(APF ? 2 * kU : 1)>(ax, av);
        };
        const int slab_it = a.slab_it;
        const int n_small = a.slab_small < n_iter ? a.slab_small : n_iter;
        const int it_small0 = n_iter - n_small;
        const int n_big = (it_small0 + slab_it - 1) / slab_it;
        n_slab = n_big + n_small;
        double *s_slab = s_stage;
        const bool lane_rec = a.slab_lane != 0;
        auto grab = [&]() {
            int v = 0;
            if (lane == 0) v = atomicAdd(&sh.next, 1);
            return __shfl_sync(0xffffffffu, v, 0);
        };
        auto first_it = [&](int sl) { return sl < n_big ? sl * slab_it : it_small0 + (sl - n_big); };
        constexpr bool PREF = (D == 1);
        int sl = grab();
        In pre;
        bool have = false;
        if (PREF && sl < n_slab && fast_ok && first_it(sl) < n_full) { load_full(first_it(sl), pre); have = true; }
        while (sl < n_slab) {
            const int i0 = first_it(sl);
            const int rem = it_small0 - i0;
            const int cnt = sl < n_big ? (rem < slab_it ? rem : slab_it) : 1;
            Acc<D> sa;
            acc_init(sa);
            Lse3 sx = lse3_empty();
            int nsl = n_slab;
            for (int k_ = 0; k_ < cnt; k_++) {
                const int i = i0 + k_;
                In cur;
                const bool cur_have = have;
                if (PREF && have) cur = pre;
                int inext = -1;
                if (k_ + 1 < cnt) inext = i + 1;
                else { nsl = grab(); if (nsl < n_slab) inext = first_it(nsl); }
                have = false;
                if (PREF && inext >= 0 && fast_ok && inext < n_full) { load_full(inext, pre); have = true; }
                if (PREF && cur_have) compute_full(i, cur, sa, sx);
                else iteration(i, sa, sx);
            }
            double *rec = s_slab + (size_t)sl * a.slab_stride;
            if (lane_rec) { rec[lane] = sa.w.m; rec[32 + lane] = sa.w.s; rec[64 + lane] = sa.w.q; }
            else warp_reduce_to_slab<D, APF>(sa, sx, mom, rec, lane);
            sl = nsl;
        }
        if (!speculate) goto step_done;
        __syncthreads();
        dec = prologue_end<APF, BS>(a, t, sh, blockIdx.x == 0, true, pc);
        if (!dec.rs) goto step_done;
        reset_c = dec.reset_c;
        acc_init(acc);
        aux = lse3_empty();
        n_slab = 0;
        if (threadIdx.x == 0) sh.next = 0;
        __syncthreads();
    }
    {
        constexpr int kBarriers = (SCHEME == SMCB_RS_MULTINOMIAL) ? 2 : 1;
        unsigned long long bar_target = (unsigned long long)gridDim.x * ((unsigned long long)dec.nrs_prev * kBarriers);
        const double *uin = a.u_in ? a.u_in + (size_t)t * (n + 1) : nullptr;
        double u_sys = 0.0;
        if (SCHEME == SMCB_RS_SYSTEMATIC) {
            if (uin) u_sys = uin[0];
            else { double u1; uniform_pair(a.key, 0ull, (uint32_t)t, kPurposeUniform, u_sys, u1); }
        }
        constexpr bool kCount = (SCHEME != SMCB_RS_MULTINOMIAL);
        const bool count_path = kCount && !a.rs_global;
        {
            LoadWeights<M, FK> load;
            load.lw = a.lw[cur];
            load.X = a.X[cur];
            load.ntot = n;
            load.m = dec.xm;
            load.s = dec.xs;
            load.model = model;
            load.kprev = kprev;
            const int64_t e1 = 2 * pend < n ? 2 * pend : n;
            if (count_path) {
                Scatter sc{a.A, (double)n, (SCHEME == SMCB_RS_SYSTEMATIC) ? u_sys : 0.0, (long long)n};
                if (threadIdx.x == 0) sh.timeout_ptr = a.sync_timeout;
                scan_scatter_groups<BS, kScanGroupWarps>(load, 2 * pstart, e1, dec.p_b, dec.p_next, a.cdf, sc,
                                                         blockIdx.x == gridDim.x - 1, sh, reinterpret_cast<int *>(s_stage),
                                                         4 * kStage);
            } else {
                scan_range<BS>(load, 2 * pstart, e1, dec.p_b, dec.p_next, a.cdf, s_warp);
            }
        }
        if (SCHEME == SMCB_RS_MULTINOMIAL) {
            spacings_pass1<BS>(a, t, sh);
            bar_target += gridDim.x;
            grid_barrier(a, bar_target);
            spacings_pass2<BS>(a, sh, s_warp);
        }
        bar_target += gridDim.x;
        grid_barrier(a, bar_target);
        auto finish_pair = [&](int64_t p, const double *X0, const double *X1, int64_t a0, int64_t a1, long long g0,
                               long long g1, bool write_A = true) {
            double xp[2][D], base[2], x[2][D];
#pragma unroll
            for (int c = 0; c < D; c++) {
                xp[0][c] = __ldg(X0 + (size_t)c * n + a0);
                xp[1][c] = __ldg(X1 + (size_t)c * n + a1);
            }
            if (APF) {
                base[0] = reset_c - model_logeta<M>(model, kprev, xp[0]);
                base[1] = reset_c - model_logeta<M>(model, kprev, xp[1]);
            } else {
                base[0] = reset_c; base[1] = reset_c;
            }
            if (write_A) {
                if (2 * p + 1 < n) *reinterpret_cast<longlong2 *>(a.A + 2 * p) = make_longlong2(g0, g1);
                else a.A[2 * p] = g0;
            }
            double l[2], av[2];
            if (zin == nullptr && vec_x && 2 * p + 1 < n) {
                double z[2][NZ];
#pragma unroll
                for (int c = 0; c < NZ; c++)
                    normal_pair_tab(a.key, (uint64_t)((a.index_offset >> 1) + p), (uint32_t)t, (uint32_t)c, z[0][c], z[1][c]);
                bool odd = false;
#pragma unroll
                for (int j2 = 0; j2 < 2; j2++) {
                    double d;
                    model_move<M, FK>(model, k, xp[j2], z[j2], x[j2], d);
                    l[j2] = base[j2] + d;
                    odd |= nonfinite(l[j2]);
                    if (APF) {
                        av[j2] = last_apf ? l[j2] + model_logeta<M>(model, k, x[j2]) : -CUDART_INF;
                        odd |= nonfinite(av[j2]);
                    }
                }
                if (odd) {
#pragma unroll
                    for (int j2 = 0; j2 < 2; j2++) { l[j2] = fix_nan(l[j2]); if (APF) av[j2] = fix_nan(av[j2]); }
                }
#pragma unroll
                for (int c = 0; c < D; c++) st2(Xo + (size_t)c * n + 2 * p, x[0][c], x[1][c]);
                st2(lwo + 2 * p, l[0], l[1]);
                if (!odd) acc_add_batch<2, D, true>(acc, l, x, mom);
                else acc_add_batch<2, D, false>(acc, l, x, mom);
            } else {
                do_pair(p, xp, base, x, l, av);
                acc_add_batch<2, D>(acc, l, x, mom);
            }
            if (APF) lse3_add_batch<2>(aux, av);
        };
        if (count_path) {
            const double M_ = (double)n;
            auto settle = [&](long long a0, double su) -> long long {
                a0 = a0 < 0 ? 0 : (a0 > n - 1 ? n - 1 : a0);
                long long lo_, hi_;
                if (__ldcg(a.cdf + a0) < su) {
                    long long step = 1;
                    lo_ = a0 + 1;
                    hi_ = a0 + 1;
                    while (hi_ < n - 1 && __ldcg(a.cdf + hi_) < su) { lo_ = hi_ + 1; hi_ += step; step <<= 1; }
                    if (hi_ > n - 1) hi_ = n - 1;
                } else {
                    long long step = 1;
                    hi_ = a0;
                    lo_ = a0 - 1;
                    while (lo_ >= 0 && __ldcg(a.cdf + lo_) >= su) { hi_ = lo_; lo_ -= step; step <<= 1; }
                    lo_ = lo_ < 0 ? 0 : lo_ + 1;
                }
                while (lo_ < hi_) {
                    const long long mid = lo_ + ((hi_ - lo_) >> 1);
                    if (__ldcg(a.cdf + mid) < su) lo_ = mid + 1; else hi_ = mid;
                }
                return lo_;
            };
            constexpr int kR = kMovePairs;
            struct Hints { long long h[kR][2]; };
            struct Cdf { double c0[kR][2], cm[kR][2], c1[kR][(SCHEME == SMCB_RS_STRATIFIED) ? 2 : 1]; };
            auto ld_hints = [&](int64_t p0, Hints &H) {
#pragma unroll
                for (int r = 0; r < kR; r++) {
                    const int64_t p = p0 + (int64_t)r * BS;
                    H.h[r][0] = H.h[r][1] = 0;
                    if (p < pend && 2 * p + 1 < n) {
                        const longlong2 hh = __ldcg(reinterpret_cast<const longlong2 *>(a.A + 2 * p));
                        H.h[r][0] = hh.x; H.h[r][1] = hh.y;
                    } else if (p < pend) {
                        H.h[r][0] = __ldcg(a.A + 2 * p);
                    }
                }
            };
            auto ld_cdf = [&](int64_t p0, const Hints &H, Cdf &Cc) {
#pragma unroll
                for (int r = 0; r < kR; r++) {
                    const int64_t p = p0 + (int64_t)r * BS;
#pragma unroll
                    for (int q = 0; q < 2; q++) {
                        long long hh = H.h[r][q];
                        hh = hh < 0 ? 0 : (hh > n - 1 ? n - 1 : hh);
                        const bool on = (p < pend) && (q == 0 || 2 * p + 1 < n);
                        Cc.c0[r][q] = on ? a.cdf[hh] : 2.0;
                        Cc.cm[r][q] = (on && hh > 0) ? a.cdf[hh - 1] : -1.0;
                        if (SCHEME == SMCB_RS_STRATIFIED) Cc.c1[r][q] = (on && hh + 1 < n) ? a.cdf[hh + 1] : 2.0;
                    }
                }
            };
            auto process = [&](int64_t p0, const Hints &H, const Cdf &Cc) {
                long long h[kR][2];
                double su[kR][2];
                bool valid[kR], two[kR], moved[kR];
#pragma unroll
                for (int r = 0; r < kR; r++) {
                    const int64_t p = p0 + (int64_t)r * BS;
                    moved[r] = false;
                    valid[r] = p < pend;
                    two[r] = valid[r] && (2 * p + 1 < n);
                    if (SCHEME == SMCB_RS_SYSTEMATIC) {
                        su[r][0] = (u_sys + (double)(2 * p)) / M_;
                        su[r][1] = (u_sys + (double)(2 * p + 1)) / M_;
                    } else {
                        double u0 = 0.0, u1 = 0.0;
                        if (valid[r]) {
                            if (uin) { u0 = uin[2 * p]; u1 = two[r] ? uin[2 * p + 1] : 0.0; }
                            else uniform_pair(a.key, (uint64_t)((a.index_offset >> 1) + p), (uint32_t)t, kPurposeUniform, u0, u1);
                        }
                        su[r][0] = (u0 + (double)(2 * p)) / M_;
                        su[r][1] = (u1 + (double)(2 * p + 1)) / M_;
                    }
#pragma unroll
                    for (int q = 0; q < 2; q++) {
                        long long hh = H.h[r][q];
                        hh = hh < 0 ? 0 : (hh > n - 1 ? n - 1 : hh);
                        moved[r] = moved[r] || hh != H.h[r][q];
                        h[r][q] = hh;
                    }
                }
#pragma unroll
                for (int r = 0; r < kR; r++) {
#pragma unroll
                    for (int q = 0; q < 2; q++) {
                        const bool on = q == 0 ? valid[r] : two[r];
                        bool ok = (Cc.cm[r][q] < su[r][q]) && (su[r][q] <= Cc.c0[r][q] || h[r][q] == n - 1);
                        if (SCHEME == SMCB_RS_STRATIFIED) {
                            if (on && !ok && Cc.c0[r][q] < su[r][q] && (su[r][q] <= Cc.c1[r][q] || h[r][q] + 1 == n - 1)) {
                                h[r][q] += 1; moved[r] = true; ok = true;
                            }
                        }
                        if (on && !ok && Cc.c0[r][q] < su[r][q] && h[r][q] + 1 < n) {
                            constexpr int kWin = 6;
                            const long long b = h[r][q] + 1;
                            double wv[kWin];
#pragma unroll
                            for (int i = 0; i < kWin; i++) wv[i] = (b + i < n) ? __ldcg(a.cdf + b + i) : 2.0;
                            int cnt = 0;
#pragma unroll
                            for (int i = 0; i < kWin; i++) cnt += (wv[i] < su[r][q]) ? 1 : 0;
                            if (cnt < kWin) {
                                long long hn = b + cnt;
                                h[r][q] = hn > n - 1 ? n - 1 : hn;
                                moved[r] = true; ok = true;
                            }
                        }
                        if (on && !ok) {
                            h[r][q] = settle(h[r][q], su[r][q]);
                            moved[r] = true;
                        }
                    }
                    if (!two[r]) h[r][1] = h[r][0];
                }
#pragma unroll
                for (int r = 0; r < kR; r++) {
                    const int64_t p = p0 + (int64_t)r * BS;
                    if (valid[r]) finish_pair(p, Xi, Xi, h[r][0], h[r][1], h[r][0], h[r][1], moved[r]);
                }
            };
            constexpr int64_t kStep = (int64_t)kR * BS;
            for (int64_t p0 = pstart + threadIdx.x; p0 < pend; p0 += kStep) {
                Hints H;
                Cdf Cc;
                ld_hints(p0, H);
                ld_cdf(p0, H, Cc);
                process(p0, H, Cc);
            }
        } else if (!a.rs_global) {
            const double M_ = (double)n;
            const double zlast = (SCHEME == SMCB_RS_MULTINOMIAL) ? __ldcg(a.su + n) : 1.0;
            int64_t lo = -1;
            if (threadIdx.x == 0) { mbar_init(&s_bar[0], 1); mbar_init(&s_bar[1], 1); mbar_init_fence(); }
            __syncthreads();
            uint32_t phase0 = 0, phase1 = 0;
            int buf = 0;
            auto issue = [&](int64_t lo_, int b) {
                const int64_t sb = lo_ & ~(int64_t)1;
                const int c = (int)((n - sb) < kStage ? (n - sb) : kStage);
                const uint32_t bytes = (uint32_t)(c & ~1) * 8u;
                double *dst = s_stage + (size_t)b * kStage;
                if (c & 1) dst[c - 1] = __ldcg(a.cdf + sb + c - 1);
                if (bytes) {
                    mbar_arrive_expect_tx(&s_bar[b], bytes);
                    tma_bulk_g2s(dst, a.cdf + sb, bytes, &s_bar[b]);
                } else {
                    mbar_arrive(&s_bar[b]);
                }
            };
            for (int64_t pbase = pstart; pbase < pend; pbase += BS) {
                const int64_t p = pbase + threadIdx.x;
                const bool active = p < pend;
                const int64_t k0 = 2 * pbase;
                const int64_t ptop = pbase + BS < pend ? pbase + BS : pend;
                const int64_t k1 = (2 * ptop < n ? 2 * ptop : n) - 1;
                double su[2] = {2.0, 2.0};
                if (active) {
                    if (SCHEME == SMCB_RS_SYSTEMATIC) {
                        su[0] = (u_sys + (double)(2 * p)) / M_;
                        su[1] = (u_sys + (double)(2 * p + 1)) / M_;
                    } else if (SCHEME == SMCB_RS_STRATIFIED) {
                        double u0, u1;
                        if (uin) { u0 = uin[2 * p]; u1 = (2 * p + 1 < n) ? uin[2 * p + 1] : 0.0; }
                        else uniform_pair(a.key, (uint64_t)((a.index_offset >> 1) + p), (uint32_t)t,
                                          kPurposeUniform, u0, u1);
                        su[0] = (u0 + (double)(2 * p)) / M_;
                        su[1] = (u1 + (double)(2 * p + 1)) / M_;
                    } else {
                        su[0] = __ldcg(a.su + 2 * p) / zlast;
                        su[1] = (2 * p + 1 < n) ? __ldcg(a.su + 2 * p + 1) / zlast : 2.0;
                    }
                    if (2 * p == k0) s_su[0] = su[0];
                    if (2 * p == k1) s_su[1] = su[0];
                    if (2 * p + 1 == k1) s_su[1] = su[1];
                }
                __syncthreads();
                const double su_first = s_su[0], su_last = s_su[1];
                if (lo < 0) {
                    lo = block_lower_bound<BS>(a.cdf, 0, n, su_first);
                    lo = lo < n - 1 ? lo : n - 1;
                    if (threadIdx.x == 0) issue(lo, buf);
                    __syncthreads();
                }
                const int64_t sbase = lo & ~(int64_t)1;
                const int cnt = (int)((n - sbase) < kStage ? (n - sbase) : kStage);
                mbar_wait(&s_bar[buf], buf ? phase1 : phase0);
                if (buf) phase1 ^= 1u; else phase0 ^= 1u;
                const double *s_cdf = s_stage + (size_t)buf * kStage;
                const bool covered = (sbase + cnt >= n) || (s_cdf[cnt - 1] >= su_last);
                int64_t hi = lo;
                if (!covered) hi = block_lower_bound<BS>(a.cdf, lo, n, su_last);
                int64_t a0 = 0, a1 = 0;
                if (active) {
                    if (covered) {
                        int l0 = (int)(lo - sbase), h0 = cnt;
                        while (l0 < h0) { const int mid = (l0 + h0) >> 1; if (s_cdf[mid] < su[0]) l0 = mid + 1; else h0 = mid; }
                        int l1 = l0, h1 = cnt;
#pragma unroll
                        for (int w = 0; w < 4; w++)
                            if (l1 < cnt && s_cdf[l1] < su[1]) l1++;
                        if (l1 < cnt && s_cdf[l1] < su[1]) {
                            while (l1 < h1) { const int mid = (l1 + h1) >> 1; if (s_cdf[mid] < su[1]) l1 = mid + 1; else h1 = mid; }
                        }
                        a0 = sbase + l0;
                        a1 = sbase + l1;
                        if (2 * p == k1) s_hi = a0;
                        if (2 * p + 1 == k1) s_hi = a1;
                    } else {
                        const int64_t hi1 = hi < n ? hi + 1 : n;
                        a0 = lower_bound_cg(a.cdf, lo, hi1, su[0]);
                        a1 = lower_bound_cg(a.cdf, a0, hi1, su[1]);
                    }
                }
                __syncthreads();
                const int64_t lo_next = covered ? (s_hi < n ? s_hi : n - 1) : (hi < n ? hi : n - 1);
                if (pbase + BS < pend && threadIdx.x == 0) issue(lo_next, buf ^ 1);
                if (active) {
                    a0 = a0 < n - 1 ? a0 : n - 1;
                    a1 = a1 < n - 1 ? a1 : n - 1;
                    finish_pair(p, Xi, Xi, a0, a1, a0, a1);
                }
                lo = lo_next;
                buf ^= 1;
            }
        } else {
            if (blockIdx.x == 0 && (int)threadIdx.x < a.world) {
                __threadfence_system();
                double *slot = a.mail_peer[threadIdx.x] + ((size_t)(t & 1) * a.world + a.rank) * kMailStride;
                *reinterpret_cast<volatile double *>(slot + kMailScan) = (double)(t + 1);
            }
            if ((int)threadIdx.x < a.world)
                wait_epoch(a.mail_local + ((size_t)(t & 1) * a.world + threadIdx.x) * kMailStride + kMailScan,
                           (double)(t + 1), a.sync_timeout);
            __syncthreads();
            const int world = a.world;
            const double M_ = (double)a.n_global;
            double *s_cdf = s_stage;
            int64_t lo = -1;
            int lo_shard = -1;
            for (int64_t pbase = pstart; pbase < pend; pbase += BS) {
                const int64_t p = pbase + threadIdx.x;
                const bool active = p < pend;
                const int64_t k0 = 2 * pbase;
                const int64_t ptop = pbase + BS < pend ? pbase + BS : pend;
                const int64_t k1 = 2 * ptop - 1;
                double su[2] = {2.0, 2.0};
                if (active) {
                    const double g0 = (double)(a.index_offset + 2 * p);
                    if (SCHEME == SMCB_RS_SYSTEMATIC) {
                        su[0] = (u_sys + g0) / M_;
                        su[1] = (u_sys + (g0 + 1.0)) / M_;
                    } else {
                        double u0, u1;
                        if (uin) { u0 = uin[2 * p]; u1 = uin[2 * p + 1]; }
                        else uniform_pair(a.key, (uint64_t)((a.index_offset >> 1) + p), (uint32_t)t, kPurposeUniform, u0, u1);
                        su[0] = (u0 + g0) / M_;
                        su[1] = (u1 + (g0 + 1.0)) / M_;
                    }
                    if (2 * p == k0) s_su[0] = su[0];
                    if (2 * p + 1 == k1) s_su[1] = su[1];
                }
                __syncthreads();
                const double su_first = s_su[0], su_last = s_su[1];
                const int kf = shard_of(sh.goff, sh.gpi, world, su_first);
                const int kl = shard_of(sh.goff, sh.gpi, world, su_last);
                int ks[2] = {kf, kf};
                int64_t an[2] = {0, 0};
                if (kf == kl) {
                    const double *cdf = a.pcdf[kf];
                    const double off = sh.goff[kf], pi = sh.gpi[kf];
                    const double v0 = fmin((su[0] - off) / pi, 1.0), v1 = fmin((su[1] - off) / pi, 1.0);
                    const double v_first = fmin((su_first - off) / pi, 1.0), v_last = fmin((su_last - off) / pi, 1.0);
                    if (lo < 0 || lo_shard != kf) lo = block_lower_bound<BS>(cdf, 0, n, v_first);
                    if (lo > n - 1) lo = n - 1;
                    lo_shard = kf;
                    const int64_t sbase = lo & ~(int64_t)1;
                    const int cnt = (int)((n - sbase) < kStage ? (n - sbase) : kStage);
                    for (int i = 2 * threadIdx.x; i < cnt; i += 2 * BS) {
                        if (i + 1 < cnt) *reinterpret_cast<double2 *>(&s_cdf[i]) = __ldcg(reinterpret_cast<const double2 *>(cdf + sbase + i));
                        else s_cdf[i] = __ldcg(cdf + sbase + i);
                    }
                    __syncthreads();
                    const bool covered = (sbase + cnt >= n) || (s_cdf[cnt - 1] >= v_last);
                    int64_t hi = lo;
                    if (!covered) hi = block_lower_bound<BS>(cdf, lo, n, v_last);
                    if (active) {
                        if (covered) {
                            int l0 = (int)(lo - sbase), h0 = cnt;
                            while (l0 < h0) { const int mid = (l0 + h0) >> 1; if (s_cdf[mid] < v0) l0 = mid + 1; else h0 = mid; }
                            int l1 = l0, h1 = cnt;
#pragma unroll
                            for (int w = 0; w < 4; w++)
                                if (l1 < cnt && s_cdf[l1] < v1) l1++;
                            if (l1 < cnt && s_cdf[l1] < v1) {
                                while (l1 < h1) { const int mid = (l1 + h1) >> 1; if (s_cdf[mid] < v1) l1 = mid + 1; else h1 = mid; }
                            }
                            an[0] = sbase + l0;
                            an[1] = sbase + l1;
                            if (2 * p + 1 == k1) s_hi = an[1];
                        } else {
                            const int64_t hi1 = hi < n ? hi + 1 : n;
                            an[0] = lower_bound_cg(cdf, lo, hi1, v0);
                            an[1] = lower_bound_cg(cdf, an[0], hi1, v1);
                        }
                    }
                    __syncthreads();
                    lo = covered ? (s_hi < n ? s_hi : n - 1) : (hi < n ? hi : n - 1);
                } else {
                    if (active) {
#pragma unroll
                        for (int j = 0; j < 2; j++) {
                            ks[j] = shard_of(sh.goff, sh.gpi, world, su[j]);
                            const double v = fmin((su[j] - sh.goff[ks[j]]) / sh.gpi[ks[j]], 1.0);
                            an[j] = lower_bound_cg(a.pcdf[ks[j]], 0, n, v);
                        }
                    }
                    lo = -1;
                }
                if (active) {
                    const int64_t a0 = an[0] < n - 1 ? an[0] : n - 1, a1 = an[1] < n - 1 ? an[1] : n - 1;
                    finish_pair(p, a.pX[ks[0]][cur], a.pX[ks[1]][cur], a0, a1, (long long)ks[0] * n + a0,
                                (long long)ks[1] * n + a1);
                }
                __syncthreads();
            }
        }
    }
step_done:
    write_partial<D, APF, BS>(a, t, acc, aux, mom, sh, s_stage, n_slab);
}

template <bool APF>
__global__ void __launch_bounds__(kTailBlock) k_tail(FilterArgs a, long long t) {
    __shared__ StepSmem sh;
    cudaGridDependencySynchronize();
    step_prologue<APF, kTailBlock>(a, t, sh, true, false);
}

template <bool APF>
__global__ void __launch_bounds__(kTailBlock) k_publish(FilterArgs a, long long s) {
    __shared__ StepSmem sh;
    double loc[16];
    shard_totals<APF>(a, s, true, sh, loc);
    if (threadIdx.x == 0)
        for (int i = 0; i < 16; i++) a.local_stats[i] = loc[i];
}

}

struct smcb_filter {
    smcb_ctx *ctx;
    smcb_filter_desc desc;
    FilterArgs args;
    char *mem;
    int grid_move;
    int block_size;
    size_t dyn_smem;
    int slab_doubles;
    int pairs_per_iteration;
    int64_t t_host;
    bool pdl, coop;
    bool timed;
    int (*launch_init)(smcb_filter *);
    int (*launch_step)(smcb_filter *);
    int (*launch_tail)(smcb_filter *);
    int (*launch_publish)(smcb_filter *);
};

template <class... Args>
static int launch_ex(smcb_filter *f, void (*kern)(Args...), int grid, int block, size_t smem, bool coop, bool pdl,
                     Args... args) {
    cudaLaunchConfig_t cfg = {};
    cfg.gridDim = dim3(grid);
    cfg.blockDim = dim3(block);
    cfg.dynamicSmemBytes = smem;
    cfg.stream = f->ctx->stream;
    cudaLaunchAttribute attr[2];
    int na = 0;
    if (coop) { attr[na].id = cudaLaunchAttributeCooperative; attr[na].val.cooperative = 1; na++; }
    if (pdl) {
        attr[na].id = cudaLaunchAttributeProgrammaticStreamSerialization;
        attr[na].val.programmaticStreamSerializationAllowed = 1;
        na++;
    }
    cfg.attrs = attr;
    cfg.numAttrs = na;
    SMCB_CUDA(cudaLaunchKernelEx(&cfg, kern, args...));
    f->ctx->launches++;
    return SMCB_OK;
}

template <class M, int FK, int SCHEME>
static int launch_step_t(smcb_filter *f) {
    M model;
    model.load(f->desc.params);
    return launch_ex(f, k_step<M, FK, SCHEME>, f->grid_move, f->block_size, f->dyn_smem, f->coop,
                     f->pdl && !f->timed, model, f->args, (long long)f->t_host);
}

template <class M, int FK>
static int launch_init_t(smcb_filter *f) {
    M model;
    model.load(f->desc.params);
    k_init<M, FK><<<f->grid_move, f->block_size, kMathTabBytes, f->ctx->stream>>>(model, f->args);
    f->ctx->launches++;
    SMCB_CUDA(cudaGetLastError());
    return SMCB_OK;
}

template <int FK>
static int launch_tail_t(smcb_filter *f) {
    return launch_ex(f, k_tail<FkTraits<FK>::apf>, 1, kTailBlock, 0, false, f->pdl && !f->timed, f->args,
                     (long long)f->t_host);
}

template <int FK>
static int launch_publish_t(smcb_filter *f) {
    k_publish<FkTraits<FK>::apf><<<1, kTailBlock, 0, f->ctx->stream>>>(f->args, (long long)(f->t_host - 1));
    f->ctx->launches++;
    SMCB_CUDA(cudaGetLastError());
    return SMCB_OK;
}

template <class M, int FK, int SCHEME>
static int bind_one(smcb_filter *f) {
    f->launch_init = launch_init_t<M, FK>;
    f->launch_step = launch_step_t<M, FK, SCHEME>;
    f->launch_tail = launch_tail_t<FK>;
    f->launch_publish = launch_publish_t<FK>;
    f->block_size = StepCfg<M>::BS;
    f->dyn_smem = StepCfg<M>::dyn_smem;
    f->slab_doubles = StepCfg<M>::kSlabDoubles;
    f->pairs_per_iteration = 32 * StepCfg<M>::kU;
    SMCB_CUDA(cudaFuncSetAttribute(k_step<M, FK, SCHEME>, cudaFuncAttributeMaxDynamicSharedMemorySize,
                                   (int)StepCfg<M>::dyn_smem));
    SMCB_CUDA(cudaFuncSetAttribute(k_init<M, FK>, cudaFuncAttributeMaxDynamicSharedMemorySize, (int)kMathTabBytes));
    int nb = 0;
    SMCB_CUDA(cudaOccupancyMaxActiveBlocksPerMultiprocessor(&nb, k_step<M, FK, SCHEME>, StepCfg<M>::BS,
                                                            StepCfg<M>::dyn_smem));
    if (nb < 1) {
        set_error("fused filter: the step kernel does not fit on an SM of this device");
        return SMCB_ECUDA;
    }
    return SMCB_OK;
}

template <class M, int FK>
static int bind_scheme(smcb_filter *f) {
    switch (f->desc.scheme) {
        case SMCB_RS_SYSTEMATIC: return bind_one<M, FK, SMCB_RS_SYSTEMATIC>(f);
        case SMCB_RS_STRATIFIED: return bind_one<M, FK, SMCB_RS_STRATIFIED>(f);
        case SMCB_RS_MULTINOMIAL: return bind_one<M, FK, SMCB_RS_MULTINOMIAL>(f);
        default:
            set_error("fused filter: resampling scheme %d is not fused (use systematic, stratified or "
                      "multinomial, or the unfused path)", f->desc.scheme);
            return SMCB_ENOSYS;
    }
}

template <class M>
static int bind_fk(smcb_filter *f) {
    switch (f->desc.fk) {
        case SMCB_FK_BOOTSTRAP: return bind_scheme<M, SMCB_FK_BOOTSTRAP>(f);
        case SMCB_FK_GUIDED:
            if (!M::has_proposal) break;
            return bind_scheme<M, SMCB_FK_GUIDED>(f);
        case SMCB_FK_APF:
            if (!M::has_proposal) break;
            return bind_scheme<M, SMCB_FK_APF>(f);
        case SMCB_FK_AUXBOOT:
            if (!M::has_proposal) break;
            return bind_scheme<M, SMCB_FK_AUXBOOT>(f);
        default:
            set_error("fused filter: unknown Feynman-Kac kind %d", f->desc.fk);
            return SMCB_EINVAL;
    }
    set_error("fused filter: model %d implements no proposal/logeta (Feynman-Kac kind %d)",
              f->desc.model, f->desc.fk);
    return SMCB_ENOSYS;
}
```

Measured before the change: 64.04 billion.

## Speculatively fuse two non-resampling SV steps into one kernel launch

When the extrapolated ESS suggests the next step will not resample, the step kernel also runs step t+1 in place, chaining particle states in registers. It stages the t+1 per-slab partials in a new global slab and writes them out, then the launch for t+1 becomes a no-op. If that step turns out to need resampling, it is flagged as mispredicted and computed normally. This removes one launch and one pass of particle reads per fused pair, at the cost of extra partial slots, a larger kernel with more register pressure, and redundant work on mispredictions.

Measured after the change: 69.61 billion, median of 6. 8.7% higher.

```diff
diff --git a/include/smcb.h b/include/smcb.h
--- a/include/smcb.h
+++ b/include/smcb.h
@@ -165,6 +165,7 @@
 int smcb_p2p_free(void *dev_ptr);
 int smcb_filter_step_timed(smcb_filter *f, int64_t nsteps, double *out8);
 int smcb_filter_state(smcb_filter *f, double *out8);
+int smcb_filter_fusion_stats(smcb_filter *f, int64_t *out3);
 
 #define SMCB_SMOOTH_ON2 0
 #define SMCB_SMOOTH_MCMC 1
diff --git a/particles_b200/_lib.py b/particles_b200/_lib.py
--- a/particles_b200/_lib.py
+++ b/particles_b200/_lib.py
@@ -102,6 +102,7 @@
     "smcb_p2p_free": (C.c_int, [C.c_void_p]),
     "smcb_filter_step_timed": (C.c_int, [C.c_void_p, C.c_int64, C.POINTER(C.c_double)]),
     "smcb_filter_state": (C.c_int, [C.c_void_p, C.POINTER(C.c_double)]),
+    "smcb_filter_fusion_stats": (C.c_int, [C.c_void_p, C.POINTER(C.c_int64)]),
     "smcb_backward_sample": (C.c_int, [C.c_void_p, C.POINTER(SmoothDesc)]),
 }
 
diff --git a/particles_b200/core.py b/particles_b200/core.py
--- a/particles_b200/core.py
+++ b/particles_b200/core.py
@@ -46,6 +46,27 @@
 
 def _is_apf(fk):
     return fk.isAPF if hasattr(fk, "isAPF") else ("logeta" in dir(fk))
+
+
+def fusion_schedule(summaries, N, ESSrmin, mode, batches):
+    table = np.asarray(summaries)
+    T = table.shape[0]
+    ess, rs_ = table[:, 0], table[:, 2] != 0
+    kinds, pre, end = [], -1, 0
+    for b in batches:
+        start, end = end, end + int(b)
+        for t in range(max(start, 1), end):
+            if pre == t:
+                kinds.append("mispredicted" if rs_[t] else "noop")
+            elif rs_[t]:
+                kinds.append("resample")
+            elif mode and t + 1 < T and t + 1 < end and (
+                    mode == 2 or 2.0 * ess[t - 1] - (ess[t - 2] if t >= 2 else ess[t - 1]) >= float(N) * ESSrmin):
+                kinds.append("fused")
+                pre = t + 1
+            else:
+                kinds.append("plain")
+    return kinds
 
 
 class _FusedEngine:
@@ -153,6 +174,11 @@
         _lib.check(self.lib.smcb_filter_state(self.handle, out))
         return list(out)
 
+    def fusion_stats(self):
+        out = (C.c_int64 * 3)()
+        _lib.check(self.lib.smcb_filter_fusion_stats(self.handle, out))
+        return dict(zip(("fused", "noop", "mispredicted"), (int(v) for v in out)))
+
     def close(self):
         if getattr(self, "handle", None):
             self.lib.smcb_filter_destroy(self.handle)
diff --git a/particles_b200/csrc/smcb_filter.cu b/particles_b200/csrc/smcb_filter.cu
--- a/particles_b200/csrc/smcb_filter.cu
+++ b/particles_b200/csrc/smcb_filter.cu
@@ -59,19 +59,8 @@
     if (rc) return rc;
 
     const int64_t n = d->n;
-    constexpr size_t kHdr = 512;
-    static_assert(2 * sizeof(StepState) <= 384, "StepState outgrew its header slot");
-    const size_t part = (size_t)2 * kMaxStepGrid * kPartStride * sizeof(double);
-    const size_t agg = (size_t)(kMaxStepGrid + 8) * sizeof(double);
-    SMCB_CUDA(cudaMalloc(&f->mem, kHdr + part + agg));
-    SMCB_CUDA(cudaMemsetAsync(f->mem, 0, kHdr + part + agg, c->stream));
     FilterArgs &a = f->args;
     memset(&a, 0, sizeof(a));
-    a.st = reinterpret_cast<StepState *>(f->mem);
-    a.bar = reinterpret_cast<unsigned long long *>(f->mem + 384);
-    a.sync_timeout = reinterpret_cast<int *>(f->mem + 392);
-    a.partials = reinterpret_cast<double *>(f->mem + kHdr);
-    a.blk_agg = reinterpret_cast<double *>(f->mem + kHdr + part);
     a.math_tab = c->math_tab;
     a.X[0] = d->X[0]; a.X[1] = d->X[1]; a.lw[0] = d->lw[0]; a.lw[1] = d->lw[1];
     a.A = reinterpret_cast<long long *>(d->A);
@@ -121,6 +110,25 @@
     }
     a.world = d->world > 1 ? d->world : 1;
     a.rank = d->world > 1 ? d->rank : 0;
+    {
+        const char *v = getenv("SMCB_FUSE");
+        const int mode = (!v || !*v) ? 1 : (v[0] == '0' ? 0 : (v[0] == '2' ? 2 : 1));
+        a.fuse_mode = (d->dim == 1 && a.world == 1) ? mode : 0;
+    }
+    constexpr size_t kHdr = 512;
+    static_assert(2 * sizeof(StepState) <= 256, "StepState outgrew its header slot");
+    const size_t part = (size_t)kPartSlots * kMaxStepGrid * kPartStride * sizeof(double);
+    const size_t agg = (size_t)(kMaxStepGrid + 8) * sizeof(double);
+    const size_t slab = a.fuse_mode ? (size_t)f->grid_move * f->slab_doubles * sizeof(double) : 0;
+    SMCB_CUDA(cudaMalloc(&f->mem, kHdr + part + agg + slab));
+    SMCB_CUDA(cudaMemsetAsync(f->mem, 0, kHdr + part + agg, c->stream));
+    a.st = reinterpret_cast<StepState *>(f->mem);
+    a.fuse = reinterpret_cast<long long *>(f->mem + 256);
+    a.bar = reinterpret_cast<unsigned long long *>(f->mem + 384);
+    a.sync_timeout = reinterpret_cast<int *>(f->mem + 392);
+    a.partials = reinterpret_cast<double *>(f->mem + kHdr);
+    a.blk_agg = reinterpret_cast<double *>(f->mem + kHdr + part);
+    a.fuse_slab = a.fuse_mode ? reinterpret_cast<double *>(f->mem + kHdr + part + agg) : nullptr;
     a.local_stats = d->local_stats;
     a.gathered = d->gathered;
     a.mail_local = (a.world > 1) ? d->mail_local : nullptr;
@@ -179,6 +187,7 @@
 extern "C" int smcb_filter_step_local(smcb_filter *f) {
     SMCB_REQUIRE(f != nullptr && f->args.world > 1 && f->args.mail_local == nullptr,
                  "smcb_filter_step_local: not a sharded filter with the host-driven exchange");
+    f->args.batch_end = f->t_host + 1;
     int rc = launch_one(f);
     if (rc) return rc;
     return f->launch_publish(f);
@@ -194,6 +203,7 @@
     SMCB_REQUIRE(f->args.world == 1 || f->args.mail_local != nullptr,
                  "smcb_filter_step: sharded filters without a peer mailbox use step_local / step_finish");
     if (nsteps <= 0) return SMCB_OK;
+    f->args.batch_end = f->t_host + nsteps;
     for (int64_t i = 0; i < nsteps; i++) {
         int rc = launch_one(f);
         if (rc) return rc;
@@ -223,6 +233,7 @@
         if (e != cudaSuccess) { fail(e, "cudaEventCreate"); break; }
     }
     f->timed = true;
+    f->args.batch_end = t_first + nsteps;
     for (int64_t i = 0; rc == SMCB_OK && i <= nsteps; i++) {
         cudaEventRecord(ev[2 * i], s);
         rc = (i < nsteps) ? launch_one(f) : f->launch_tail(f);
@@ -282,6 +293,15 @@
     return SMCB_OK;
 }
 
+extern "C" int smcb_filter_fusion_stats(smcb_filter *f, int64_t *out3) {
+    SMCB_REQUIRE(f && out3, "smcb_filter_fusion_stats: NULL argument");
+    long long h[4];
+    SMCB_CUDA(cudaMemcpyAsync(h, f->args.fuse, sizeof(h), cudaMemcpyDeviceToHost, f->ctx->stream));
+    SMCB_CUDA(cudaStreamSynchronize(f->ctx->stream));
+    for (int i = 0; i < 3; i++) out3[i] = h[1 + i];
+    return SMCB_OK;
+}
+
 extern "C" int smcb_p2p_alloc(smcb_ctx *c, int64_t bytes, void **dev_ptr, unsigned char *handle64) {
     SMCB_REQUIRE(c && dev_ptr && handle64 && bytes > 0, "smcb_p2p_alloc: bad argument");
     static_assert(sizeof(cudaIpcMemHandle_t) == 64, "IPC handle size");
diff --git a/particles_b200/csrc/smcb_step.cuh b/particles_b200/csrc/smcb_step.cuh
--- a/particles_b200/csrc/smcb_step.cuh
+++ b/particles_b200/csrc/smcb_step.cuh
@@ -2,6 +2,7 @@
 #include <string.h>
 
 #include <new>
+#include <type_traits>
 
 #include "smcb_common.cuh"
 #include "smcb_math.cuh"
@@ -20,6 +21,7 @@
 constexpr int kMaxStepGrid = 256;
 constexpr int kMaxD = 4;
 constexpr int kTailBlock = 256;
+constexpr int kPartSlots = 4;
 #ifndef SMCB_SPECULATE
 #define SMCB_SPECULATE 1
 #endif
@@ -58,6 +60,10 @@
     StepState *st;
     int *sync_timeout;
     double *partials;
+    int fuse_mode;
+    int64_t batch_end;
+    long long *fuse;
+    double *fuse_slab;
     unsigned long long *bar;
     double *blk_agg;
     const double *math_tab;
@@ -323,7 +329,7 @@
         v[0] = w4[0]; v[1] = w4[1]; v[2] = w4[2]; v[3] = w4[3];
     }
     if (threadIdx.x == 0) {
-        double *p = a.partials + ((size_t)(t & 1) * kMaxStepGrid + blockIdx.x) * kPartStride;
+        double *p = a.partials + ((size_t)(t % kPartSlots) * kMaxStepGrid + blockIdx.x) * kPartStride;
         p[0] = mx[0]; p[1] = v[0]; p[2] = v[1]; p[3] = 0.0;
         p[4] = APF ? mx[1] : mx[0]; p[5] = APF ? v[2] : v[0]; p[6] = APF ? v[3] : v[1]; p[7] = 0.0;
 #pragma unroll
@@ -354,7 +360,7 @@
 __device__ __forceinline__ void shard_totals(const FilterArgs &a, long long s, bool mom, StepSmem &sh, double (&loc)[16]) {
     const int G = a.grid, tid = threadIdx.x;
     if (tid < 32) {
-        const double *base = a.partials + (size_t)(s & 1) * kMaxStepGrid * kPartStride;
+        const double *base = a.partials + (size_t)(s % kPartSlots) * kMaxStepGrid * kPartStride;
         constexpr int kR = kMaxStepGrid / 32;
         double pm[kR], ps[kR], pq[kR], xm[kR], xs[kR], xq[kR];
         double mw = -CUDART_INF, ma = -CUDART_INF;
@@ -438,6 +444,7 @@
     double reset_c;
     double xm, xs;
     double p_b, p_next;
+    double ess;
 };
 
 struct PrologueCarry {
@@ -543,6 +550,7 @@
     d.reset_c = rc;
     d.xm = xl.m; d.xs = xl.s;
     d.p_b = 0.0; d.p_next = 0.0;
+    d.ess = ess;
     if (writer && tid == 0) {
         double *row = a.summaries + (size_t)s * SMCB_SUMMARY_STRIDE;
         row[0] = ess; row[1] = logLt; row[2] = (double)rs_s; row[3] = log_mean;
@@ -563,7 +571,7 @@
     if (d.rs && need_prefix) {
         double v = 0.0;
         if (tid < a.grid) {
-            const double *row = a.partials + ((size_t)(s & 1) * kMaxStepGrid + tid) * kPartStride + (APF ? 4 : 0);
+            const double *row = a.partials + ((size_t)(s % kPartSlots) * kMaxStepGrid + tid) * kPartStride + (APF ? 4 : 0);
             v = __ldcg(row + 1) * shift_factor(__ldcg(row), d.xm) / d.xs;
         }
         cta_prefix<BS>(v, sh, d.p_b, d.p_next);
@@ -953,6 +961,25 @@
     return k;
 }
 
+struct StepIo {
+    long long t;
+    StepK k;
+    const double *zin;
+    double *Xo, *lwo;
+    bool last_apf;
+};
+
+__device__ __forceinline__ StepIo step_io(const FilterArgs &a, long long t, int nz) {
+    StepIo io;
+    io.t = t;
+    io.k = step_consts(a, t);
+    io.zin = a.z_in ? a.z_in + (size_t)t * nz * a.n : nullptr;
+    io.Xo = a.X[t & 1];
+    io.lwo = a.lw[t & 1];
+    io.last_apf = t + 1 < a.T;
+    return io;
+}
+
 template <class M, int FK, int SCHEME>
 __global__ void __launch_bounds__(StepCfg<M>::BS, 1) k_step(M model, FilterArgs a, long long t) {
     constexpr bool APF = FkTraits<FK>::apf;
@@ -974,20 +1001,32 @@
     const bool speculate = SMCB_SPECULATE && a.world > 1 && a.mail_local != nullptr && !a.rs_global && !pred_rs;
     StepDecision dec;
     dec.rs = 0; dec.nrs_prev = 0; dec.reset_c = 0.0; dec.xm = 0.0; dec.xs = 1.0; dec.p_b = 0.0; dec.p_next = 0.0;
+    dec.ess = 0.0;
     if (!speculate) dec = prologue_end<APF, BS>(a, t, sh, blockIdx.x == 0, true, pc);
     mbar_wait(&s_tabbar, 0);
     const int cur = (int)((t - 1) & 1);
     const bool rs = dec.rs != 0;
+    if (a.fuse_mode != 0 && __ldcg(a.fuse) == t) {
+        if (blockIdx.x == 0 && threadIdx.x == 0) a.fuse[rs ? 3 : 2] += 1;
+        if (!rs) return;
+    }
+    bool fuse = false;
+    if (D == 1 && !rs && a.fuse_mode != 0 && a.world == 1 && t + 1 < a.T && t + 1 < a.batch_end) {
+        const double ess2 = (t >= 2) ? __ldcg(&a.st[(t - 2) & 1].ess) : dec.ess;
+        fuse = a.fuse_mode == 2 || 2.0 * dec.ess - ess2 >= (double)a.n_global * a.essrmin;
+    }
+    if (fuse && blockIdx.x == 0 && threadIdx.x == 0) { a.fuse[0] = t + 1; a.fuse[1] += 1; }
     double reset_c = dec.reset_c;
-    const StepK k = step_consts(a, t);
+    const StepIo io0 = step_io(a, t, NZ);
+    const StepK &k = io0.k;
     const StepK kprev = step_consts(a, t - 1);
     const double *__restrict__ Xi = a.X[cur];
     const double *__restrict__ lwi = a.lw[cur];
-    double *__restrict__ Xo = a.X[cur ^ 1];
-    double *__restrict__ lwo = a.lw[cur ^ 1];
+    double *__restrict__ Xo = io0.Xo;
+    double *__restrict__ lwo = io0.lwo;
     const int64_t n = a.n;
-    const double *zin = a.z_in ? a.z_in + (size_t)t * NZ * n : nullptr;
-    const bool last_apf = APF && (t + 1 < a.T);
+    const double *zin = io0.zin;
+    const bool last_apf = APF && io0.last_apf;
     const bool mom = a.moments != nullptr;
     const bool vec_x = (D == 1) || ((n & 1) == 0);
     int64_t pstart, pend;
@@ -998,40 +1037,40 @@
     Lse3 aux = lse3_empty();
     int n_slab = 0;
 
-    auto do_pair = [&](int64_t p, const double (&xp)[2][D], const double (&base)[2], double (&x)[2][D], double *l,
-                       double *av) {
+    auto do_pair = [&](const StepIo &io, int64_t p, const double (&xp)[2][D], const double (&base)[2],
+                       double (&x)[2][D], double *l, double *av) {
         double z[2][NZ];
 #pragma unroll
         for (int c = 0; c < NZ; c++) {
-            if (zin) {
-                const double *zz = zin + (size_t)c * n;
+            if (io.zin) {
+                const double *zz = io.zin + (size_t)c * n;
                 z[0][c] = zz[2 * p];
                 z[1][c] = (2 * p + 1 < n) ? zz[2 * p + 1] : 0.0;
             } else {
-                normal_pair_tab(a.key, (uint64_t)((a.index_offset >> 1) + p), (uint32_t)t, (uint32_t)c,
+                normal_pair_tab(a.key, (uint64_t)((a.index_offset >> 1) + p), (uint32_t)io.t, (uint32_t)c,
                                  z[0][c], z[1][c]);
             }
         }
 #pragma unroll
         for (int j = 0; j < 2; j++) {
             double d;
-            model_move<M, FK>(model, k, xp[j], z[j], x[j], d);
+            model_move<M, FK>(model, io.k, xp[j], z[j], x[j], d);
             l[j] = fix_nan(base[j] + d);
-            if (APF) av[j] = last_apf ? fix_nan(l[j] + model_logeta<M>(model, k, x[j])) : -CUDART_INF;
+            if (APF) av[j] = io.last_apf ? fix_nan(l[j] + model_logeta<M>(model, io.k, x[j])) : -CUDART_INF;
         }
         if (2 * p + 1 < n) {
             if (vec_x) {
 #pragma unroll
-                for (int c = 0; c < D; c++) st2(Xo + (size_t)c * n + 2 * p, x[0][c], x[1][c]);
+                for (int c = 0; c < D; c++) st2(io.Xo + (size_t)c * n + 2 * p, x[0][c], x[1][c]);
             } else {
 #pragma unroll
-                for (int c = 0; c < D; c++) { Xo[(size_t)c * n + 2 * p] = x[0][c]; Xo[(size_t)c * n + 2 * p + 1] = x[1][c]; }
-            }
-            st2(lwo + 2 * p, l[0], l[1]);
+                for (int c = 0; c < D; c++) { io.Xo[(size_t)c * n + 2 * p] = x[0][c]; io.Xo[(size_t)c * n + 2 * p + 1] = x[1][c]; }
+            }
+            st2(io.lwo + 2 * p, l[0], l[1]);
         } else {
 #pragma unroll
-            for (int c = 0; c < D; c++) { Xo[(size_t)c * n + 2 * p] = x[0][c]; x[1][c] = 0.0; }
-            lwo[2 * p] = l[0];
+            for (int c = 0; c < D; c++) { io.Xo[(size_t)c * n + 2 * p] = x[0][c]; x[1][c] = 0.0; }
+            io.lwo[2 * p] = l[0];
             l[1] = -CUDART_INF;
             if (APF) av[1] = -CUDART_INF;
         }
@@ -1048,25 +1087,24 @@
         const bool fast_ok = (zin == nullptr) && vec_x;
         const double *__restrict__ lwi_c = lwi + 2 * pstart;
         const double *__restrict__ Xi_c = Xi + 2 * pstart;
-        double *__restrict__ lwo_c = lwo + 2 * pstart;
-        double *__restrict__ Xo_c = Xo + 2 * pstart;
         const uint64_t gpair0 = (uint64_t)((a.index_offset >> 1) + pstart);
         struct In { double base[kU][2]; double xp[kU][2][D]; };
-        auto load_full = [&](int i, In &in) {
+        auto load_full = [&](const double *Xs_c, const double *lws_c, int i, In &in) {
 #pragma unroll
             for (int u = 0; u < kU; u++) {
                 const int o2 = 2 * (i * kIt + u * 32 + lane);
-                const double2 tl = ld2(lwi_c + o2);
+                const double2 tl = ld2(lws_c + o2);
                 in.base[u][0] = tl.x; in.base[u][1] = tl.y;
 #pragma unroll
                 for (int c = 0; c < D; c++) {
-                    const double2 tx = ld2(Xi_c + (size_t)c * n + o2);
+                    const double2 tx = ld2(Xs_c + (size_t)c * n + o2);
                     in.xp[u][0][c] = tx.x; in.xp[u][1][c] = tx.y;
                 }
             }
         };
-        auto compute_full = [&](int i, const In &in, Acc<D> &ac, Lse3 &ax) {
-            double l[2 * kU], av[APF ? 2 * kU : 1], x[2 * kU][D];
+        auto compute_full = [&](const StepIo &io, int i, const In &in, Acc<D> &ac, Lse3 &ax, double (&l)[2 * kU],
+                                double (&x)[2 * kU][D]) {
+            double av[APF ? 2 * kU : 1];
             bool odd = false;
 #pragma unroll
             for (int u = 0; u < kU; u++) {
@@ -1074,16 +1112,16 @@
                 double z[2][NZ];
 #pragma unroll
                 for (int c = 0; c < NZ; c++)
-                    normal_pair_tab(a.key, gpair0 + (uint64_t)prel, (uint32_t)t, (uint32_t)c, z[0][c], z[1][c]);
+                    normal_pair_tab(a.key, gpair0 + (uint64_t)prel, (uint32_t)io.t, (uint32_t)c, z[0][c], z[1][c]);
 #pragma unroll
                 for (int j2 = 0; j2 < 2; j2++) {
                     double d;
-                    model_move<M, FK>(model, k, in.xp[u][j2], z[j2], x[2 * u + j2], d);
+                    model_move<M, FK>(model, io.k, in.xp[u][j2], z[j2], x[2 * u + j2], d);
                     l[2 * u + j2] = in.base[u][j2] + d;
                     odd |= nonfinite(l[2 * u + j2]);
                     if (APF) {
-                        av[APF ? 2 * u + j2 : 0] = last_apf ? l[2 * u + j2] + model_logeta<M>(model, k, x[2 * u + j2])
-                                                            : -CUDART_INF;
+                        av[APF ? 2 * u + j2 : 0] = io.last_apf ? l[2 * u + j2] + model_logeta<M>(model, io.k, x[2 * u + j2])
+                                                               : -CUDART_INF;
                         odd |= nonfinite(av[APF ? 2 * u + j2 : 0]);
                     }
                 }
@@ -1095,6 +1133,8 @@
                     if (APF) av[APF ? q : 0] = fix_nan(av[APF ? q : 0]);
                 }
             }
+            double *const lwo_c = io.lwo + 2 * pstart;
+            double *const Xo_c = io.Xo + 2 * pstart;
 #pragma unroll
             for (int u = 0; u < kU; u++) {
                 const int o2 = 2 * (i * kIt + u * 32 + lane);
@@ -1109,42 +1149,39 @@
             }
             if (APF) lse3_add_batch<(APF ? 2 * kU : 1)>(ax, av);
         };
-        auto iteration = [&](int i, Acc<D> &ac, Lse3 &ax) {
-            double l[2 * kU], av[APF ? 2 * kU : 1], x[2 * kU][D];
-            if (fast_ok && i < n_full) {
-                In in;
-                load_full(i, in);
-                compute_full(i, in, ac, ax);
-                return;
-            }
-            double xp[kU][2][D], base[kU][2];
+        auto load_general = [&](const double *Xs, const double *lws, int i, In &in) {
             const int64_t qbase = pstart + (int64_t)i * kIt;
 #pragma unroll
             for (int u = 0; u < kU; u++) {
                 const int64_t p = qbase + u * 32 + lane;
                 if (p < pend && 2 * p + 1 < n) {
-                    double2 tl = ld2(lwi + 2 * p);
-                    base[u][0] = tl.x; base[u][1] = tl.y;
+                    double2 tl = ld2(lws + 2 * p);
+                    in.base[u][0] = tl.x; in.base[u][1] = tl.y;
 #pragma unroll
                     for (int c = 0; c < D; c++) {
                         if (vec_x) {
-                            double2 tx = ld2(Xi + (size_t)c * n + 2 * p);
-                            xp[u][0][c] = tx.x; xp[u][1][c] = tx.y;
+                            double2 tx = ld2(Xs + (size_t)c * n + 2 * p);
+                            in.xp[u][0][c] = tx.x; in.xp[u][1][c] = tx.y;
                         } else {
-                            xp[u][0][c] = Xi[(size_t)c * n + 2 * p]; xp[u][1][c] = Xi[(size_t)c * n + 2 * p + 1];
+                            in.xp[u][0][c] = Xs[(size_t)c * n + 2 * p]; in.xp[u][1][c] = Xs[(size_t)c * n + 2 * p + 1];
                         }
                     }
                 } else if (p < pend) {
-                    base[u][0] = lwi[2 * p]; base[u][1] = 0.0;
-#pragma unroll
-                    for (int c = 0; c < D; c++) { xp[u][0][c] = Xi[(size_t)c * n + 2 * p]; xp[u][1][c] = 0.0; }
-                }
-            }
+                    in.base[u][0] = lws[2 * p]; in.base[u][1] = 0.0;
+#pragma unroll
+                    for (int c = 0; c < D; c++) { in.xp[u][0][c] = Xs[(size_t)c * n + 2 * p]; in.xp[u][1][c] = 0.0; }
+                }
+            }
+        };
+        auto compute_general = [&](const StepIo &io, int i, const In &in, Acc<D> &ac, Lse3 &ax, double (&l)[2 * kU],
+                                   double (&x)[2 * kU][D]) {
+            double av[APF ? 2 * kU : 1];
+            const int64_t qbase = pstart + (int64_t)i * kIt;
 #pragma unroll
             for (int u = 0; u < kU; u++) {
                 const int64_t p = qbase + u * 32 + lane;
                 if (p < pend) {
-                    do_pair(p, xp[u], base[u], reinterpret_cast<double (&)[2][D]>(x[2 * u]), l + 2 * u,
+                    do_pair(io, p, in.xp[u], in.base[u], reinterpret_cast<double (&)[2][D]>(x[2 * u]), l + 2 * u,
                             APF ? av + 2 * u : av);
                 } else {
                     l[2 * u] = l[2 * u + 1] = -CUDART_INF;
@@ -1161,7 +1198,6 @@
         const int it_small0 = n_iter - n_small;
         const int n_big = (it_small0 + slab_it - 1) / slab_it;
         n_slab = n_big + n_small;
-        double *s_slab = s_stage;
         const bool lane_rec = a.slab_lane != 0;
         auto grab = [&]() {
             int v = 0;
@@ -1169,36 +1205,80 @@
             return __shfl_sync(0xffffffffu, v, 0);
         };
         auto first_it = [&](int sl) { return sl < n_big ? sl * slab_it : it_small0 + (sl - n_big); };
-        constexpr bool PREF = (D == 1);
-        int sl = grab();
-        In pre;
-        bool have = false;
-        if (PREF && sl < n_slab && fast_ok && first_it(sl) < n_full) { load_full(first_it(sl), pre); have = true; }
-        while (sl < n_slab) {
-            const int i0 = first_it(sl);
-            const int rem = it_small0 - i0;
-            const int cnt = sl < n_big ? (rem < slab_it ? rem : slab_it) : 1;
-            Acc<D> sa;
-            acc_init(sa);
-            Lse3 sx = lse3_empty();
-            int nsl = n_slab;
-            for (int k_ = 0; k_ < cnt; k_++) {
-                const int i = i0 + k_;
-                In cur;
-                const bool cur_have = have;
-                if (PREF && have) cur = pre;
-                int inext = -1;
-                if (k_ + 1 < cnt) inext = i + 1;
-                else { nsl = grab(); if (nsl < n_slab) inext = first_it(nsl); }
-                have = false;
-                if (PREF && inext >= 0 && fast_ok && inext < n_full) { load_full(inext, pre); have = true; }
-                if (PREF && cur_have) compute_full(i, cur, sa, sx);
-                else iteration(i, sa, sx);
-            }
-            double *rec = s_slab + (size_t)sl * a.slab_stride;
+        auto park = [&](double *rec, const Acc<D> &sa, const Lse3 &sx) {
             if (lane_rec) { rec[lane] = sa.w.m; rec[32 + lane] = sa.w.s; rec[64 + lane] = sa.w.q; }
             else warp_reduce_to_slab<D, APF>(sa, sx, mom, rec, lane);
-            sl = nsl;
+        };
+        constexpr bool PREF = (D == 1);
+        auto slabs = [&](auto fused) {
+            constexpr bool FUSED = decltype(fused)::value;
+            constexpr bool PF = PREF && !FUSED;
+            const StepIo io1 = FUSED ? step_io(a, t + 1, NZ) : io0;
+            const double *Xs = FUSED ? a.X[cur] : Xi;
+            const double *lws = FUSED ? a.lw[cur] : lwi;
+            const double *Xs_c = FUSED ? Xs + 2 * pstart : Xi_c;
+            const double *lws_c = FUSED ? lws + 2 * pstart : lwi_c;
+            double *const slab1 = FUSED ? a.fuse_slab + (size_t)blockIdx.x * StepCfg<M>::kSlabDoubles : nullptr;
+            int sl = grab();
+            In pre;
+            bool have = false;
+            if (PF && sl < n_slab && fast_ok && first_it(sl) < n_full) {
+                load_full(Xs_c, lws_c, first_it(sl), pre);
+                have = true;
+            }
+            while (sl < n_slab) {
+                const int i0 = first_it(sl);
+                const int rem = it_small0 - i0;
+                const int cnt = sl < n_big ? (rem < slab_it ? rem : slab_it) : 1;
+                Acc<D> sa, sb;
+                acc_init(sa);
+                Lse3 sx = lse3_empty(), sy = lse3_empty();
+                if (FUSED) acc_init(sb);
+                int nsl = n_slab;
+                for (int k_ = 0; k_ < cnt; k_++) {
+                    const int i = i0 + k_;
+                    In cin;
+                    const bool cur_have = have;
+                    if (PF && have) cin = pre;
+                    int inext = -1;
+                    if (k_ + 1 < cnt) inext = i + 1;
+                    else { nsl = grab(); if (nsl < n_slab) inext = first_it(nsl); }
+                    have = false;
+                    if (PF && inext >= 0 && fast_ok && inext < n_full) { load_full(Xs_c, lws_c, inext, pre); have = true; }
+                    const bool full = fast_ok && i < n_full;
+                    if (!(PF && cur_have)) {
+                        if (full) load_full(Xs_c, lws_c, i, cin);
+                        else load_general(Xs, lws, i, cin);
+                    }
+                    double l[2 * kU], x[2 * kU][D];
+                    if (full) compute_full(io0, i, cin, sa, sx, l, x);
+                    else compute_general(io0, i, cin, sa, sx, l, x);
+                    if (FUSED) {
+                        In nx;
+#pragma unroll
+                        for (int u = 0; u < kU; u++) {
+#pragma unroll
+                            for (int j2 = 0; j2 < 2; j2++) {
+                                nx.base[u][j2] = l[2 * u + j2];
+#pragma unroll
+                                for (int c = 0; c < D; c++) nx.xp[u][j2][c] = x[2 * u + j2][c];
+                            }
+                            if (!full && 2 * (pstart + (int64_t)i * kIt + u * 32 + lane) + 1 == n) nx.base[u][1] = 0.0;
+                        }
+                        if (full) compute_full(io1, i, nx, sb, sy, l, x);
+                        else compute_general(io1, i, nx, sb, sy, l, x);
+                    }
+                }
+                park(s_stage + (size_t)sl * a.slab_stride, sa, sx);
+                if (FUSED) park(slab1 + (size_t)sl * a.slab_stride, sb, sy);
+                sl = nsl;
+            }
+        };
+        if constexpr (D == 1) {
+            if (fuse) slabs(std::true_type{});
+            else slabs(std::false_type{});
+        } else {
+            slabs(std::false_type{});
         }
         if (!speculate) goto step_done;
         __syncthreads();
@@ -1296,7 +1376,7 @@
                 if (!odd) acc_add_batch<2, D, true>(acc, l, x, mom);
                 else acc_add_batch<2, D, false>(acc, l, x, mom);
             } else {
-                do_pair(p, xp, base, x, l, av);
+                do_pair(io0, p, xp, base, x, l, av);
                 acc_add_batch<2, D>(acc, l, x, mom);
             }
             if (APF) lse3_add_batch<2>(aux, av);
@@ -1634,6 +1714,9 @@
     }
 step_done:
     write_partial<D, APF, BS>(a, t, acc, aux, mom, sh, s_stage, n_slab);
+    if (fuse)
+        write_partial<D, APF, BS>(a, t + 1, acc, aux, mom, sh, a.fuse_slab + (size_t)blockIdx.x * StepCfg<M>::kSlabDoubles,
+                                  n_slab);
 }
 
 template <bool APF>
```
